# luoao-kddi/SCP

Hardware: AMD Instinct MI355X
Metric: KITTI frames/sec encode (SCP-EHEM, level 16) + bpp match vs ref (higher is better)
Workload: dtype f32 (dense layers and attention as bf16x3 split on bf16 MFMA, feature kNN as f16x3 split on f16 MFMA, fp32 accumulate; position kNN / CDF in fp32); 1 GPU; SCP-EHEM KITTI-like synthetic 120k-pt frames, --spher --mullevel lidar_level=16 (BASELINE.json configs[2]), seeded random weights; nodes_per_frame=577403, windows_per_frame=100, frames_per_gpu=46, frames_in_flight=4, frames_per_launch_sequence=1, transform=host-numpy on a prefetch thread (strict identity: the reference's integers), parallelism=frame-sharded x1, rank_cores=256, rank_cores_pinned=False

## Files before the change

include/scp.h:

```cpp
#ifndef SCP_H
#define SCP_H
#include <stddef.h>
#include <stdint.h>

#ifdef __cplusplus
extern "C" {
#endif

#define SCP_API __attribute__((visibility("default")))

#define SCP_OK 0
#define SCP_EINVAL (-1)
#define SCP_ENOMEM (-2)
#define SCP_ESMALL (-3)
#define SCP_EHIP (-4)
#define SCP_ESTATE (-5)

#define SCP_MAX_DEPTH 21
#define SCP_MAX_SEGMENTS 62

#define SCP_ABI_VERSION 220
SCP_API int scp_version(void);
SCP_API int scp_last_hip_error(void);
SCP_API int scp_device_count(void);
// ... 68 lines not shown
                                      uint8_t *sym_coded, int64_t *pos_mm, void *stream);

SCP_API int scp_geom_context_octattn(scp_geom *g, int32_t seg, uint8_t *ctx, float *pos, uint8_t *sym, void *stream);

SCP_API int scp_knn_topk(const float *x, int32_t B, int32_t n, int32_t C, int32_t k, int32_t *idx, void *stream);

SCP_API int scp_knn_topk_packed(const float *x, const int32_t *ctab, int32_t total_rows, int32_t C, int32_t *idx, void *stream);
SCP_API int scp_knn_topk_packed_bounded(const float *x, const int32_t *ctab, int32_t total_rows, int32_t C, const float *thr0,
                                int32_t *idx, void *stream);

SCP_API int scp_edge_gather_max(const float *u, const float *v, const int32_t *idx, const float *scale, const float *shift,
                        int32_t B, int32_t n, int32_t Cout, int32_t k, float *out, int32_t out_stride, void *stream);
SCP_API int scp_edge_gather_max_ld(const float *u, int64_t ldu, const float *v, int64_t ldv, const int32_t *idx, const float *scale,
                           const float *shift, int32_t B, int32_t n, int32_t Cout, int32_t k, float *out, int32_t out_stride,
                           void *stream);

SCP_API int scp_swin_attention(const float *q, const float *k, const float *v, const float *bias_table,
                       int32_t B, int32_t Lp, int32_t shift, int32_t ldq, int32_t ldkv, float *out, void *stream);

SCP_API int scp_split_weight_bf16(const float *W, int32_t N, int32_t K, int32_t Npad, int32_t Kpad, void *hi, void *lo, void *stream);
SCP_API int scp_linear_bf16x3(const float *A, int64_t lda, const void *Whi, const void *Wlo, int32_t Kpad, const float *bias,
                      const float *residual, int64_t ldr, float *C, int64_t ldc, int32_t M, int32_t N, int32_t K, int32_t act,
                      void *stream);

SCP_API int scp_split_weight_f16(const float *W, int32_t N, int32_t K, int32_t Npad, int32_t Kpad, void *hi, void *lo,
                                 float *inv_scale, void *stream);
SCP_API int scp_linear_f16x3(const float *A, int64_t lda, const void *Whi, const void *Wlo, const float *w_inv_scale, int32_t Kpad,
                             const float *bias, const float *residual, int64_t ldr, float *C, int64_t ldc, int32_t M, int32_t N,
                             int32_t K, int32_t act, float *row_scale_ws, void *stream);
SCP_API int scp_row_scale_f16(const float *A, int64_t lda, int32_t M, int32_t K, float *scale, float *inv_scale, void *stream);
SCP_API int scp_linear_f16x3_scaled(const float *A, int64_t lda, const void *Whi, const void *Wlo, const float *w_inv_scale, int32_t Kpad,
                                    const float *bias, const float *residual, int64_t ldr, float *C, int64_t ldc, int32_t M, int32_t N,
                                    int32_t K, int32_t act, const float *scale, const float *inv_scale, void *stream);

SCP_API int scp_tile_weight_bf16(const void *plane, int32_t Npad, int32_t Kpad, void *tiled, void *stream);
SCP_API int scp_split_rows_f16(const float *A, int64_t lda, int32_t M, int32_t K, void *hi, void *lo, int64_t ldp, float *scale, float *inv_scale,
                               void *stream);
SCP_API int scp_layernorm_add_split_f16(const float *a, const float *b, int64_t rows, int32_t C, const float *gamma, const float *beta, float eps,
                                        float *out, void *hi, void *lo, int64_t ldp, float *scale, float *inv_scale, void *stream);
SCP_API int scp_linear_split_f16(const void *Ahi, const void *Alo, int64_t lda, const float *a_inv_scale, const void *Whi, const void *Wlo,
                                 const float *w_inv_scale, int32_t Npad, int32_t Kpad, const float *bias, const float *residual, int64_t ldr,
                                 float *C, int64_t ldc, int32_t M, int32_t N, int32_t K, int32_t act, int32_t cfg, void *stream);
SCP_API int scp_linear_split_f16_max(const void *Ahi, const void *Alo, int64_t lda, const float *a_inv_scale, const void *Whi, const void *Wlo,
                                     const float *w_inv_scale, int32_t Npad, int32_t Kpad, const float *bias, const float *residual, int64_t ldr,
                                     float *C, int64_t ldc, int32_t M, int32_t N, int32_t K, int32_t act, int32_t cfg, uint32_t *row_max,
                                     uint32_t *col_max, int32_t col_lo, int32_t col_hi, int32_t col_rows, void *stream);
SCP_API int scp_row_scale_from_max(const uint32_t *row_max, int32_t M, float *scale, float *inv_scale, void *stream);
SCP_API int scp_linear_split(const void *Ahi, const void *Alo, int64_t lda, const void *Whi, const void *Wlo, int32_t Npad, int32_t Kpad,
                     const float *bias, const float *residual, int64_t ldr, float *C, int64_t ldc, void *Ohi, void *Olo, int64_t ldo,
                     int32_t M, int32_t N, int32_t K, int32_t act, int32_t cfg, void *stream);

SCP_API int scp_linear_split_gather(const void *Ahi, const void *Alo, int64_t lda, const void *Whi, const void *Wlo, int32_t Npad, int32_t Kpad,
                            const float *bias, const float *residual, int64_t ldr, const int64_t *res_map, float *C, int64_t ldc, void *Ohi,
                            void *Olo, int64_t ldo, int32_t M, int32_t N, int32_t K, int32_t act, int32_t cfg, void *stream);
SCP_API int scp_linear_split_hier2(const void *A0hi, const void *A0lo, int64_t lda0, int32_t K0pad, const void *A1hi, const void *A1lo, int64_t lda1,
                                   int64_t M1, const void *W0hi, const void *W0lo, const void *W1hi, const void *W1lo, int32_t Npad,
                                   const int64_t *parent, const float *bias, const float *res, int64_t ldr, const int64_t *res_map, void *Ohi,
                                   void *Olo, int64_t ldo, int32_t M, int32_t N, int32_t act, void *stream);
SCP_API int scp_linear_split_scatter(const void *Ahi, const void *Alo, int64_t lda, const void *Whi, const void *Wlo, int32_t Npad, int32_t Kpad,
                             const float *bias, const int64_t *out_map, float *C, int64_t ldc, int32_t M, int32_t N, int32_t K, int32_t act,
                             int32_t cfg, void *stream);
SCP_API int scp_split_rows(const float *src, int64_t ld_src, int64_t n_src, const int64_t *idx, int32_t C, void *hi, void *lo, int64_t ldo,
                   int64_t rows, void *stream);
SCP_API int scp_layernorm_rows_split(const float *x, int64_t ldx, int64_t n_src_rows, const int64_t *ia, const int64_t *ib, int32_t C,
                             const float *gamma, const float *beta, const float *valid, float eps, void *ohi, void *olo, int64_t ldo,
                             int64_t rows, void *stream);
SCP_API int scp_layernorm_add(const float *a, const float *b, int64_t rows, int32_t C, const float *gamma, const float *beta, float eps,
                              float *out, void *stream);
SCP_API int scp_swin_attention_packed_split(const float *q, const float *k, const float *v, const float *bias_table, const int32_t *wtab,
                                    int32_t total_windows, int32_t shift, int32_t ldq, int32_t ldkv, void *ohi, void *olo, int64_t ldo,
                                    void *stream);


SCP_API int scp_swin_attention_packed(const float *q, const float *k, const float *v, const float *bias_table, const int32_t *wtab,
                              int32_t total_windows, int32_t shift, int32_t ldq, int32_t ldkv, float *out, void *stream);

SCP_API int scp_layernorm_rows(const float *x, int64_t ldx, int64_t n_src_rows, const int64_t *ia, const int64_t *ib, int32_t C,
                       const float *gamma, const float *beta, const float *valid, float eps, float *out, int64_t ldo, int64_t rows,
                       void *stream);
SCP_API int scp_gather_rows(const float *src, int64_t lds, const int64_t *idx, int32_t C, float *out, int64_t ldo, int64_t rows, void *stream);

SCP_API int scp_linear_f32(const float *A, int64_t lda, const float *W, const float *bias, float *C, int64_t ldc, int32_t M, int32_t N, int32_t K,
                   int32_t act, void *stream);

SCP_API int scp_octattn_attention(const float *q_u, const float *k, const float *k_u, const float *v, const float *v_u,
                          int32_t B, int32_t c, int32_t H, int32_t hd, float *out, float *out_u, void *stream);

SCP_API int64_t scp_octattn_f16x3_ws_bytes(int32_t B, int32_t c, int32_t H);
SCP_API int scp_octattn_attention_f16x3(const float *q_u, const float *k, const float *k_u, const float *v, const float *v_u,
                                        int64_t ldkv, int32_t B, int32_t c, int32_t H, int32_t hd, float *out, float *out_u, void *workspace,
                                        int64_t ws_bytes, void *stream);
SCP_API int scp_octattn_attention_f16x3_vmax(const float *q_u, const float *k, const float *k_u, const float *v, const float *v_u,
                                             int64_t ldkv, int32_t B, int32_t c, int32_t H, int32_t hd, float *out, float *out_u, void *workspace,
                                             int64_t ws_bytes, const uint32_t *vmax_bits, void *stream);
SCP_API int scp_octattn_attention_rowinv(const float *q_u, int64_t qw, int64_t qr, const float *k, const float *v, int64_t kw, int64_t kr,
                                         const float *k_u, const float *v_u, int64_t uw, int64_t ur, float *out, float *out_u, int64_t ow,
                                         int64_t orr, int32_t B, int32_t q0, int32_t q1, int32_t qoff, int32_t H, int32_t hd, void *stream);
SCP_API int scp_octattn_attention_rowinv_step(const float *q_u, int64_t qr, const float *k, const float *v, int64_t kw, int64_t kr,
                                              int32_t slots, int32_t rows, const float *k_u, const float *v_u, int64_t ur, float *out,
                                              float *out_u, int64_t orr, const int32_t *t, const int32_t *slot, int32_t S, int32_t H,
                                              int32_t hd, void *stream);
SCP_API int scp_decode_expand_octattn(const int64_t *sym, const int64_t *cum, const uint8_t *ctx, const int32_t *apos, int64_t n, int32_t L,
                                      int32_t shift, int32_t depth, uint8_t *cctx, int32_t *capos, float *cpos, uint8_t *occ8, void *stream);
SCP_API int scp_octattn_embed(const uint8_t *ctx, const float *pos, int64_t n, int32_t c, const float *occ_enc, int32_t d_occ,
                              const float *level_enc, int32_t d_lvl, int32_t max_level, const float *octant_enc, int32_t d_oct,
                              const float *pos_w, const float *pos_b, int32_t d_pos, const float *pe, int32_t level_cap, float *E,
                              void *hi, void *lo, int64_t ldp, float *scale, float *inv_scale, void *stream);

SCP_API int scp_softmax_cdf(const float *logits, int64_t ld, int64_t n, int32_t nsym, const uint8_t *sym,
                    float *pmf, uint32_t *lohi, uint16_t *cdf_full, void *stream);
SCP_API int scp_pmf_cdf(const float *pmf, int64_t n, int32_t nsym, const uint8_t *sym, uint32_t *lohi,
                uint16_t *cdf_full, void *stream);

typedef struct scp_rate_seg {
    int64_t rows;
    double ideal_bits, table_bits;
    int64_t top1, bad_rows;
} scp_rate_seg;
SCP_API int64_t scp_rate_workspace_bytes(int64_t n, int32_t nseg);
SCP_API int scp_rate_segments(const float *logits, int64_t ld, int64_t n, int32_t nsym, const uint8_t *sym, const uint32_t *lohi,
                              const int64_t *seg_off, int32_t nseg, scp_rate_seg *out, double *row_ideal, double *row_table,
                              void *workspace, int64_t workspace_bytes, void *stream);

SCP_API int scp_ac_encode_cdf(const uint16_t *cdf, const int16_t *sym, int64_t n, int32_t Lp, uint8_t *out, size_t cap,
                      size_t *out_len);
SCP_API int scp_ac_encode_lohi(const uint32_t *lohi, int64_t n, uint8_t *out, size_t cap, size_t *out_len);
typedef struct scp_ac_dec scp_ac_dec;
SCP_API int scp_ac_dec_new(scp_ac_dec **d, const uint8_t *stream, size_t len, int32_t Lp);
SCP_API int scp_ac_dec_next(scp_ac_dec *d, const uint16_t *cdf_row);
SCP_API int scp_ac_dec_run(scp_ac_dec *d, const uint16_t *cdf, int64_t n, int16_t *out);
SCP_API int scp_ac_dec_free(scp_ac_dec *d);

typedef struct scp_legacy_node { uint32_t nodeid, octant, parent; uint8_t oct; uint32_t pos[3]; } scp_legacy_node;
SCP_API void *new_vector(void);
SCP_API void delete_vector(void *v);
SCP_API int vector_size(void *v);
SCP_API void *vector_get(void *v, int level);
SCP_API void vector_push_back(void *v, int i);
SCP_API void *genOctreeInterface(void *v, const double *xyz, int n);
SCP_API int Nodes_size(void *level);
SCP_API scp_legacy_node *Nodes_get(void *level, int i);
SCP_API int int_size(void *codes);
SCP_API int int_get(void *codes, int i);

SCP_API int scp_nn_sqdist_f64(const double *a, int64_t na, const double *b, int64_t nb, double *d2, void *stream);

enum { SCP_TIE_MEAN_NORMAL = 0, SCP_TIE_PLANE_ERROR = 1 };
SCP_API int scp_estimate_normals_f64(const double *xyz, int64_t n, double radius, int32_t max_nn, const double *view, double *normals,
                                     int32_t *count, int32_t *idx, void *stream);
SCP_API int scp_nn_tieset_f64(int32_t mode, const double *q, int64_t nq, const double *p, int64_t np, const double *dmin, const double *nrm,
                              double *out, void *stream);

#define SCP_DIST_MAX_RINGS 64
#define SCP_DIST_MAX_BINS 4096
#define SCP_DIST_MAX_POINTS (1ll << 30)
enum { SCP_DIST_FLAG_AXIS = 1, SCP_DIST_FLAG_GROUP_CLAMPED = 2, SCP_DIST_FLAG_NO_NEIGHBOUR = 4 };
typedef struct scp_dist_seg {
    int64_t rows, axis_rows;
    double sum_sq, sum_r2, sum_phi2, sum_theta2, sum_r, max_sq;
    int64_t hist[64];
} scp_dist_seg;
SCP_API int scp_nn_error_split_f64(const double *a, int64_t na, const double *b, int64_t nb, const double *view, const double *edges_sq,
                                   int32_t n_rings, const int32_t *group , int32_t n_groups, int32_t *idx_out, double *d2_out,
                                   double *comp_out , int32_t *bin_out, uint8_t *flag_out, void *stream);
SCP_API int scp_dist_segments_f64(const double *d2, const double *comp, const uint8_t *flag, const int64_t *order , int64_t n,
                                  const int64_t *seg_off, int32_t n_bins, scp_dist_seg *out, void *stream);

#define SCP_SHARE_MAX_NODES (1ll << 30)
typedef struct scp_share_seg {
    int64_t leaves;
    double ideal_bits, table_bits, max_ideal_bits;
} scp_share_seg;
SCP_API int64_t scp_rate_leaf_share_workspace_bytes(int64_t total_nodes, int32_t nseg);
SCP_API int scp_rate_leaf_share(const uint8_t *occ, const uint8_t *level, const int32_t *parent, int64_t total_nodes, const double *bits_ideal,
                                const double *bits_table, const int64_t *segs , int32_t nseg, int64_t total_leaves,
                                int64_t *leaves, double *cost_ideal, double *cost_table, void *workspace, int64_t workspace_bytes, void *stream);
SCP_API int scp_ring_bins_f64(const double *xyz, int64_t n, const double *view, const double *edges_sq, int32_t n_rings,
                              const int32_t *group , int32_t n_groups, int32_t *bin_out, uint8_t *flag_out , void *stream);
SCP_API int scp_share_segments_f64(const double *cost_ideal, const double *cost_table, const int64_t *order , int64_t n,
                                   const int64_t *seg_off, int32_t n_bins, scp_share_seg *out, void *stream);

SCP_API int scp_embed_gather(const uint8_t *ctx, const float *pos, const int64_t *inmap, int64_t n_tokens, const float *occ_enc,
                     const float *level_enc, const float *octant_enc, float *x, float *pos_out, int64_t *occ_self, int64_t rows,
                     void *stream);

SCP_API int scp_packed_plan_sizes(const int64_t *lengths, int32_t W, int64_t *rows_out);
SCP_API int scp_packed_plan(const int64_t *lengths, int32_t W, int64_t *tables_dev, void *const *outs, int32_t n_outs, void *stream);

SCP_API int scp_decode_expand(const int64_t *sym, const int64_t *cum, const int32_t *pos, const uint8_t *anc, const uint8_t *octant, int64_t n,
                              int32_t L, int32_t shift, int32_t lv_next, int32_t lv_clamp, int32_t polar, double mn, double den, int32_t *cpos,
                              uint8_t *canc, uint8_t *coct, uint8_t *cctx, float *cposn, uint8_t *occ8, void *stream);

typedef struct scp_expand_seg {
    int64_t first, count, cfirst, coded;
    int32_t L, shift, lv_next, lv_clamp, polar, reserved;
    double mn, den;
} scp_expand_seg;
SCP_API int scp_decode_expand_batch(const int64_t *sym, const int64_t *cum, const int32_t *pos, const uint8_t *anc, const uint8_t *octant,
                                    int64_t n, const scp_expand_seg *seg, int32_t S, int32_t cs, const int64_t *wbase, int32_t K, int64_t M,
                                    int64_t T, void *table_dev, int32_t *cpos, uint8_t *canc, uint8_t *coct, uint8_t *cctx, float *cposn,
                                    uint8_t *occ8, void *stream);

SCP_API int scp_swin_ln_linear(const float *x, int64_t ldx, const float *valid, const void *Whi, const void *Wlo, const float *bias,
                               const float *wbeta, float eps, float *out, int64_t ldo, int32_t M, int32_t N, void *stream);
SCP_API int scp_swin_post_attn(const void *Ohi, const void *Olo, int64_t ldo_in, const float *x, int64_t ldx, const void *W, const float *bp,
                               const float *b1, const float *b2, float eps, float *out, int64_t ldc, int32_t M, const int32_t *tile_list,
                               int32_t n_tiles, void *stream);
SCP_API int64_t scp_swin_post_attn_weight_bytes(void);
SCP_API double scp_gelu_prescale(void);

SCP_API int scp_swin_merge(const float *x, int64_t ldx, int64_t n_src, const int64_t *ia, const int64_t *ib, const void *W, const float *wbeta,
                           float eps, float *out, int64_t ldo, int32_t M, void *stream);

SCP_API int scp_geo_edge_mlps(const float *pos1, int64_t ld1, const float *pos2, int64_t ld2, const float *pos3, int64_t ld3, const void *W,
                              const float *bias, float *out, int64_t ldo, int32_t M, void *stream);
SCP_API int scp_mlp3_rows(const float *x, int64_t ldx, int64_t n_src, const int64_t *in_map, const void *W, const float *bias, float *out, int64_t ldo,
                          const int64_t *out_map, int32_t M, int32_t N, void *stream);

SCP_API int scp_swin_kv_planes(const float *k, const float *v, int64_t ldkv, int64_t rows, void *khi, void *klo, void *vthi, void *vtlo, void *stream);
SCP_API int scp_swin_ln_qkv(const float *x, int64_t ldx, const float *valid, const void *Whi, const void *Wlo, const float *bias, const float *wbeta,
                            float eps, float *q, int64_t ldq, void *planes, int64_t Tp, int32_t M, int32_t N, void *stream);
SCP_API int scp_swin_attention_packed_planes(const float *q, const void *khi, const void *klo, const void *vthi, const void *vtlo,
                                             const float *bias_table, const int32_t *wtab, int32_t total_windows, int32_t shift, int32_t ldq,
                                             float *out, void *ohi, void *olo, int64_t ldo, const float *valid, void *stream);

#ifdef __cplusplus
}
#endif
#endif
```

include/scp_debug.h:

```cpp
#ifndef SCP_DEBUG_H
#define SCP_DEBUG_H
#include "scp.h"

#ifdef __cplusplus
extern "C" {
#endif

SCP_API int scp_set_knn_mode(int32_t f16x3);
SCP_API int scp_set_attention_mode(int32_t bf16x3);

SCP_API int scp_set_knn_workgroup(int32_t shape);
SCP_API int scp_knn_debug_buffer(unsigned long long *dev_buf);
SCP_API int scp_rc_debug_buffer(unsigned long long *dev_buf);
SCP_API int scp_set_attention_variant(int32_t v);
SCP_API int scp_get_attention_variant(void);
SCP_API int scp_rc_set_grid(int32_t workgroups);
SCP_API int scp_rc_set_wide(int32_t mode);

enum {
    SCP_PROF_POST_ATTN = 1,
    SCP_PROF_LN_LINEAR = 2,
    SCP_PROF_ATTENTION = 3,
    SCP_PROF_KNN_FEAT = 4,
    SCP_PROF_KNN_POS = 5,
    SCP_PROF_GEMM_SPLIT = 6,
    SCP_PROF_EDGE_MLP = 7,
    SCP_PROF_MERGE = 8,
    SCP_PROF_EDGE_GATHER = 9,
    SCP_PROF_CDF = 10,
    SCP_PROF_GEMM_F32 = 11,
    SCP_PROF_GEMM_ROWS = 12,
    SCP_PROF_SPLIT_ROWS = 13,
    SCP_PROF_LAYERNORM = 14,
    SCP_PROF_OA_ATTENTION = 15,
    SCP_PROF_GEOM = 16,
    SCP_PROF_OTHER = 17,
    SCP_PROF_MLP3 = 18,
    SCP_PROF_RATE = 19,
    SCP_PROF_NTAGS = 20
};
SCP_API int scp_prof_enable(int32_t on);
SCP_API int scp_prof_count(void);
SCP_API int scp_prof_read(int32_t cap, int32_t *tags, float *ms, double *work);

#ifdef __cplusplus
}
#endif
#endif
```

scp_amd/csrc/fused.hip:

```cpp
#include "scp_internal.h"

typedef _Float16 sf16x4 __attribute__((ext_vector_type(4)));
typedef float f32x4 __attribute__((ext_vector_type(4)));
typedef __bf16 bf16x4 __attribute__((ext_vector_type(4)));

template <int NV>
__global__ __launch_bounds__(256) void layernorm_rows_kernel(const float *__restrict__ x, int64_t ldx, int64_t n_src_rows,
                                                            const int64_t *__restrict__ ia, const int64_t *__restrict__ ib,
                                                            const float *__restrict__ gamma, const float *__restrict__ beta,
                                                            const float *__restrict__ valid, float eps, float *__restrict__ out, int64_t ldo,
                                                            int64_t rows, __bf16 *__restrict__ ohi, __bf16 *__restrict__ olo) {
    constexpr int RPW = 4;
    constexpr int C = 256 * NV;
    const int lane = threadIdx.x & 63;
    const int64_t r0 = ((int64_t)blockIdx.x * 4 + (threadIdx.x >> 6)) * RPW;
    if (r0 >= rows) return;
    f32x4 v[RPW][NV];
#pragma unroll
    for (int i = 0; i < RPW; ++i) {
        const int64_t r = r0 + i < rows ? r0 + i : rows - 1;
#pragma unroll
        for (int p = 0; p < NV; ++p) {
            int64_t src = r;
            if (ia) src = (p == 0) ? ia[r] : ib[r];
// ... 124 lines not shown
            if (lane + 64 * p < nq) mx = fmaxf(fmaxf(mx, fmaxf(fabsf(v[p][0]), fabsf(v[p][1]))), fmaxf(fabsf(v[p][2]), fabsf(v[p][3])));
        for (int o = 32; o > 0; o >>= 1) mx = fmaxf(mx, __shfl_xor(mx, o));
        float sc, isc;
        scp_pow2_scale(mx, sc, isc);
        if (lane == 0) { psc[r] = sc; pisc[r] = isc; }
        const int nqp = ((C + 31) & ~31) >> 2;
#pragma unroll
        for (int p = 0; p < NP; ++p) {
            const int q = lane + 64 * p;
            if (q >= nqp) continue;
            sf16x4 h4, l4;
#pragma unroll
            for (int u = 0; u < 4; ++u) {
                const float x = (q < nq ? v[p][u] : 0.f) * sc;
                const _Float16 hh = (_Float16)x;
                h4[u] = hh;
                l4[u] = (_Float16)(x - (float)hh);
            }
            *(sf16x4 *)(phi + r * ldp + 4 * q) = h4;
            *(sf16x4 *)(plo + r * ldp + 4 * q) = l4;
        }
    }
}

extern "C" SCP_API int scp_layernorm_add(const float *a, const float *b, int64_t rows, int32_t C, const float *gamma, const float *beta, float eps,
                                         float *out, void *stream) {
    if (!a || !gamma || !beta || !out || rows < 0 || C <= 0 || (C & 3) || C > 1024 ||
        (((uintptr_t)a | (uintptr_t)b | (uintptr_t)out | (uintptr_t)gamma | (uintptr_t)beta) & 15))
        return SCP_EINVAL;
    if (rows == 0) return SCP_OK;
    const unsigned nb = (unsigned)cdiv64(rows, 4);
    hipStream_t st = (hipStream_t)stream;
    SCP_PROF(SCP_PROF_LAYERNORM, st, (b ? 12.0 : 8.0) * rows * C);
    if (C <= 256) hipLaunchKernelGGL(layernorm_add_kernel<1>, dim3(nb), dim3(256), 0, st, a, b, rows, C, gamma, beta, eps, out);
    else if (C <= 512) hipLaunchKernelGGL(layernorm_add_kernel<2>, dim3(nb), dim3(256), 0, st, a, b, rows, C, gamma, beta, eps, out);
    else if (C <= 768) hipLaunchKernelGGL(layernorm_add_kernel<3>, dim3(nb), dim3(256), 0, st, a, b, rows, C, gamma, beta, eps, out);
    else hipLaunchKernelGGL(layernorm_add_kernel<4>, dim3(nb), dim3(256), 0, st, a, b, rows, C, gamma, beta, eps, out);
    LAUNCH_CHECK();
    return SCP_OK;
}

extern "C" SCP_API int scp_layernorm_add_split_f16(const float *a, const float *b, int64_t rows, int32_t C, const float *gamma, const float *beta,
                                                   float eps, float *out, void *hi, void *lo, int64_t ldp, float *scale, float *inv_scale,
                                                   void *stream) {
    const int Cp = (C + 31) & ~31;
    if (!a || !gamma || !beta || !out || !hi || !lo || !scale || !inv_scale || rows < 0 || C <= 0 || (C & 3) || Cp > 1024 || ldp < Cp || (ldp & 7) ||
        (((uintptr_t)a | (uintptr_t)b | (uintptr_t)out | (uintptr_t)gamma | (uintptr_t)beta | (uintptr_t)hi | (uintptr_t)lo) & 15))
        return SCP_EINVAL;
    if (rows == 0) return SCP_OK;
    const unsigned nb = (unsigned)cdiv64(rows, 4);
    hipStream_t st = (hipStream_t)stream;
    SCP_PROF(SCP_PROF_LAYERNORM, st, (b ? 16.0 : 12.0) * rows * C);
#define GOP(NP_) hipLaunchKernelGGL((layernorm_add_kernel<NP_, true>), dim3(nb), dim3(256), 0, st, a, b, rows, C, gamma, beta, eps, out, (_Float16 *)hi, \
                                    (_Float16 *)lo, ldp, scale, inv_scale)
    if (Cp <= 256) GOP(1); else if (Cp <= 512) GOP(2); else if (Cp <= 768) GOP(3); else GOP(4);
#undef GOP
    LAUNCH_CHECK();
    return SCP_OK;
}

__global__ __launch_bounds__(256) void gather_rows_kernel(const float *__restrict__ src, int64_t lds, const int64_t *__restrict__ idx, int C4,
                                                         float *__restrict__ out, int64_t ldo, int64_t total ) {
    const int64_t g = (int64_t)blockIdx.x * 256 + threadIdx.x;
    if (g >= total) return;
    const int64_t r = g / C4;
    const int c = (int)(g - r * C4) * 4;
    *(f32x4 *)(out + r * ldo + c) = *(const f32x4 *)(src + idx[r] * lds + c);
}

extern "C" SCP_API int scp_gather_rows(const float *src, int64_t lds, const int64_t *idx, int32_t C, float *out, int64_t ldo, int64_t rows,
                                       void *stream) {
    if (!src || !idx || !out || rows < 0 || C <= 0 || (C & 3) || (lds & 3) || (ldo & 3) || (((uintptr_t)src | (uintptr_t)out) & 15)) return SCP_EINVAL;
    if (rows == 0) return SCP_OK;
    const int64_t total = rows * (C / 4);
    hipLaunchKernelGGL(gather_rows_kernel, dim3((unsigned)cdiv64(total, 256)), dim3(256), 0, (hipStream_t)stream, src, lds, idx, C / 4, out, ldo,
                       total);
    LAUNCH_CHECK();
    return SCP_OK;
}

__global__ __launch_bounds__(256) void embed_gather_kernel(const unsigned char *__restrict__ ctx, const float *__restrict__ pos,
                                                          const int64_t *__restrict__ inmap, int64_t n_tokens, const float *__restrict__ occ_enc,
                                                          const float *__restrict__ level_enc, const float *__restrict__ octant_enc,
                                                          float *__restrict__ x, float *__restrict__ pos_out, int64_t *__restrict__ occ_self,
                                                          int64_t rows) {
    const int64_t g = (int64_t)blockIdx.x * 256 + threadIdx.x;
    if (g >= rows * 20) return;
    const int64_t r = g / 20;
    const int p = (int)(g - r * 20);
    const int64_t t = inmap[r];
    const bool pad = t >= n_tokens;
    const unsigned char *c = ctx + (pad ? 0 : t) * 12;
    f32x4 v;
    if (p < 12) {
        const int a = p >> 2;
        const int occ = pad ? 255 : c[3 * a + 2];
        v = *(const f32x4 *)(occ_enc + occ * 16 + 4 * (p & 3));
    } else if (p < 16) {
        const int lv = pad ? 0 : c[3 * (p - 12)];
        v = *(const f32x4 *)(level_enc + lv * 4);
    } else {
        const int oc = pad ? 0 : c[3 * (p - 16) + 1];
        v = *(const f32x4 *)(octant_enc + oc * 4);
    }
    *(f32x4 *)(x + r * 80 + 4 * p) = v;
    if (p == 0) {
        occ_self[r] = pad ? 255 : c[11];
        pos_out[3 * r] = pad ? 0.f : pos[3 * t];
        pos_out[3 * r + 1] = pad ? 0.f : pos[3 * t + 1];
        pos_out[3 * r + 2] = pad ? 0.f : pos[3 * t + 2];
    }
}

extern "C" SCP_API int scp_embed_gather(const uint8_t *ctx, const float *pos, const int64_t *inmap, int64_t n_tokens, const float *occ_enc,
                                        const float *level_enc, const float *octant_enc, float *x, float *pos_out, int64_t *occ_self,
                                        int64_t rows, void *stream) {
    if (!ctx || !pos || !inmap || !occ_enc || !level_enc || !octant_enc || !x || !pos_out || !occ_self || rows < 0 || n_tokens <= 0 ||
        (((uintptr_t)occ_enc | (uintptr_t)level_enc | (uintptr_t)octant_enc | (uintptr_t)x) & 15))
        return SCP_EINVAL;
    if (rows == 0) return SCP_OK;
    hipLaunchKernelGGL(embed_gather_kernel, dim3((unsigned)cdiv64(rows * 20, 256)), dim3(256), 0, (hipStream_t)stream, ctx, pos, inmap, n_tokens,
                       occ_enc, level_enc, octant_enc, x, pos_out, occ_self, rows);
    LAUNCH_CHECK();
    return SCP_OK;
}
```

scp_amd/csrc/gemm.hip:

```cpp
#include "scp_internal.h"

typedef __bf16 bf16x8 __attribute__((ext_vector_type(8)));
typedef __bf16 bf16x4 __attribute__((ext_vector_type(4)));
typedef _Float16 f16x8 __attribute__((ext_vector_type(8)));
typedef _Float16 f16x4 __attribute__((ext_vector_type(4)));
typedef float f32x16 __attribute__((ext_vector_type(16)));
typedef float f32x4 __attribute__((ext_vector_type(4)));

#define BM 128
#define BN 128
#define BK 32
#define LDP 40

enum { ACT_NONE = 0, ACT_LEAKY = 1, ACT_GELU = 2, ACT_RELU = 3 };

template <int act>
__device__ __forceinline__ float apply_act(float y) {
    if (act == ACT_LEAKY) return y > 0.f ? y : 0.01f * y;
    if (act == ACT_GELU) return scp_gelu(y);
    if (act == ACT_RELU) return y > 0.f ? y : 0.f;
    return y;
}

template <int ACT, bool F16>
// ... 295 lines not shown
            }
            *(f16x4 *)(hi + (int64_t)(row0 + i) * ldp + k) = h4;
            *(f16x4 *)(lo + (int64_t)(row0 + i) * ldp + k) = l4;
        }
    }
}

extern "C" SCP_API int scp_split_rows_f16(const float *A, int64_t lda, int32_t M, int32_t K, void *hi, void *lo, int64_t ldp, float *scale,
                                          float *inv_scale, void *stream) {
    const int Kp = (K + 31) & ~31;
    if (!A || !hi || !lo || !scale || !inv_scale || M <= 0 || K <= 0 || (K & 3) || K > 1024 || (lda & 3) || lda < K || ldp < Kp || (ldp & 7) ||
        ((uintptr_t)A & 15) || (((uintptr_t)hi | (uintptr_t)lo) & 15))
        return SCP_EINVAL;
    const dim3 grid((unsigned)((M + 15) / 16));
    SCP_PROF(SCP_PROF_SPLIT_ROWS, stream, 8.0 * M * (double)K);
#define GOR(N_) hipLaunchKernelGGL((split_rows_f16_kernel<N_>), grid, dim3(256), 0, (hipStream_t)stream, A, lda, M, K, Kp, (_Float16 *)hi, (_Float16 *)lo, \
                                   ldp, scale, inv_scale)
    if (Kp <= 256) GOR(1); else if (Kp <= 512) GOR(2); else if (Kp <= 768) GOR(3); else GOR(4);
#undef GOR
    LAUNCH_CHECK();
    return SCP_OK;
}

__global__ __launch_bounds__(256) void row_scale_from_max_kernel(const unsigned *__restrict__ mxb, int M, float *__restrict__ sc, float *__restrict__ isc) {
    const int m = blockIdx.x * 256 + threadIdx.x;
    if (m >= M) return;
    float s, is;
    pow2_scale(__uint_as_float(mxb[m]), s, is);
    sc[m] = s; isc[m] = is;
}

extern "C" SCP_API int scp_row_scale_from_max(const uint32_t *row_max, int32_t M, float *scale, float *inv_scale, void *stream) {
    if (!row_max || !scale || !inv_scale || M <= 0) return SCP_EINVAL;
    hipLaunchKernelGGL(row_scale_from_max_kernel, dim3((unsigned)((M + 255) / 256)), dim3(256), 0, (hipStream_t)stream, (const unsigned *)row_max, M, scale, inv_scale);
    LAUNCH_CHECK();
    return SCP_OK;
}

extern "C" SCP_API int scp_row_scale_f16(const float *A, int64_t lda, int32_t M, int32_t K, float *scale, float *inv_scale, void *stream) {
    if (!A || !scale || !inv_scale || M <= 0 || K <= 0 || (K & 3) || (lda & 3) || lda < K || ((uintptr_t)A & 15)) return SCP_EINVAL;
    hipLaunchKernelGGL(row_scale_kernel, dim3((unsigned)((M + 15) / 16)), dim3(256), 0, (hipStream_t)stream, A, lda, M, K, scale, inv_scale);
    LAUNCH_CHECK();
    return SCP_OK;
}

static int linear_f16x3_launch(const float *A, int64_t lda, const void *Whi, const void *Wlo, const float *w_inv_scale, int32_t Kpad,
                               const float *bias, const float *residual, int64_t ldr, float *C, int64_t ldc, int32_t M, int32_t N, int32_t K,
                               int32_t act, float *sc, float *isc, bool compute_scales, void *stream) {
    if (!A || !Whi || !Wlo || !w_inv_scale || !C || !sc || !isc || M <= 0 || N <= 0 || K <= 0 || (K & 3) || (lda & 3) || Kpad < K ||
        (Kpad % BK) || act < 0 || act > 3 || ((uintptr_t)A & 15) || lda < K || ldc < N || (residual && ldr < N))
        return SCP_EINVAL;
    if (compute_scales) hipLaunchKernelGGL(row_scale_kernel, dim3((unsigned)((M + 15) / 16)), dim3(256), 0, (hipStream_t)stream, A, lda, M, K, sc, isc);
    const dim3 grid((unsigned)(((N + BN - 1) / BN) * ((M + BM - 1) / BM)));
    SCP_PROF(SCP_PROF_GEMM_ROWS, stream, 2.0 * M * (double)N * K);
#define GO(ACT) hipLaunchKernelGGL((gemm_bf16x3_kernel<ACT, true>), grid, dim3(512), 0, (hipStream_t)stream, A, lda, (const __bf16 *)Whi, \
                              (const __bf16 *)Wlo, Kpad, bias, residual, ldr, C, ldc, M, N, K, sc, isc, w_inv_scale, gemm_wtiled())
    switch (act) { case ACT_LEAKY: GO(ACT_LEAKY); break; case ACT_GELU: GO(ACT_GELU); break; case ACT_RELU: GO(ACT_RELU); break; default: GO(ACT_NONE); }
#undef GO
    LAUNCH_CHECK();
    return SCP_OK;
}

extern "C" SCP_API int scp_linear_f16x3(const float *A, int64_t lda, const void *Whi, const void *Wlo, const float *w_inv_scale,
                                        int32_t Kpad, const float *bias, const float *residual, int64_t ldr, float *C, int64_t ldc,
                                        int32_t M, int32_t N, int32_t K, int32_t act, float *row_scale_ws, void *stream) {
    if (!row_scale_ws) return SCP_EINVAL;
    return linear_f16x3_launch(A, lda, Whi, Wlo, w_inv_scale, Kpad, bias, residual, ldr, C, ldc, M, N, K, act, row_scale_ws, row_scale_ws + M, true,
                               stream);
}

extern "C" SCP_API int scp_linear_f16x3_scaled(const float *A, int64_t lda, const void *Whi, const void *Wlo, const float *w_inv_scale,
                                               int32_t Kpad, const float *bias, const float *residual, int64_t ldr, float *C, int64_t ldc,
                                               int32_t M, int32_t N, int32_t K, int32_t act, const float *scale, const float *inv_scale,
                                               void *stream) {
    return linear_f16x3_launch(A, lda, Whi, Wlo, w_inv_scale, Kpad, bias, residual, ldr, C, ldc, M, N, K, act, (float *)scale, (float *)inv_scale,
                               false, stream);
}

#define FBM 128
#define FBN 64
#define FBK 32
#define FLD 36

template <int ACT>
__global__ __launch_bounds__(256, 2) void gemm_f32_kernel(const float *__restrict__ A, int64_t lda, const float *__restrict__ W,
                                                         const float *__restrict__ bias, float *__restrict__ C, int64_t ldc, int M, int N, int K) {
    __shared__ __attribute__((aligned(16))) float sA[FBM * FLD];
    __shared__ __attribute__((aligned(16))) float sB[FBN * FLD];
    const int tid = threadIdx.x, w = tid >> 6, lane = tid & 63, col = lane & 31, h = lane >> 5;
    const int ntn = (N + FBN - 1) / FBN;
    const int m0 = (blockIdx.x / ntn) * FBM, n0 = (blockIdx.x % ntn) * FBN;
    f32x16 acc[2];
#pragma unroll
    for (int j = 0; j < 2; ++j)
#pragma unroll
        for (int r = 0; r < 16; ++r) acc[j][r] = 0.f;
    const int nk = (K + FBK - 1) / FBK;
    const bool vec = ((K & 3) == 0) && ((lda & 3) == 0) && ((((uintptr_t)A | (uintptr_t)W) & 15) == 0);
    const int pr = tid >> 3, pc = (tid & 7) * 4;
    f32x4 ra[4], rb[2];
    auto load_tile = [&](int kt) {
        const int kk = kt * FBK + pc;
        const bool kin = kk < K;
#pragma unroll
        for (int i = 0; i < 4; ++i) {
            const int m = m0 + pr + 32 * i;
            const int mc = m < M ? m : M - 1, kc = kin ? kk : 0;
            const f32x4 v = *(const f32x4 *)(A + (int64_t)mc * lda + kc);
            ra[i] = (kin && m < M) ? v : (f32x4){0.f, 0.f, 0.f, 0.f};
        }
#pragma unroll
        for (int i = 0; i < 2; ++i) {
            const int n = n0 + pr + 32 * i;
            const int nc = n < N ? n : N - 1, kc = kin ? kk : 0;
            const f32x4 v = *(const f32x4 *)(W + (int64_t)nc * K + kc);
            rb[i] = (kin && n < N) ? v : (f32x4){0.f, 0.f, 0.f, 0.f};
        }
    };
    auto store_tile = [&]() {
        const int o = pc >> 1;
#pragma unroll
        for (int i = 0; i < 4; ++i) {
            float *d = sA + (pr + 32 * i) * FLD;
            *(float2 *)(d + o) = make_float2(ra[i][0], ra[i][2]);
            *(float2 *)(d + 16 + o) = make_float2(ra[i][1], ra[i][3]);
        }
#pragma unroll
        for (int i = 0; i < 2; ++i) {
            float *d = sB + (pr + 32 * i) * FLD;
            *(float2 *)(d + o) = make_float2(rb[i][0], rb[i][2]);
            *(float2 *)(d + 16 + o) = make_float2(rb[i][1], rb[i][3]);
        }
    };
    if (vec) load_tile(0);
    for (int kt = 0; kt < nk; ++kt) {
        const int k0 = kt * FBK;
        __syncthreads();
        if (vec) {
            store_tile();
        } else {
        for (int e = tid; e < FBM * FBK; e += 256) {
            const int r = e >> 5, k = e & 31;
            const int m = m0 + r, kk = k0 + k;
            sA[r * FLD + (k & 1) * 16 + (k >> 1)] = (m < M && kk < K) ? A[(int64_t)m * lda + kk] : 0.f;
        }
        for (int e = tid; e < FBN * FBK; e += 256) {
            const int r = e >> 5, k = e & 31;
            const int n = n0 + r, kk = k0 + k;
            sB[r * FLD + (k & 1) * 16 + (k >> 1)] = (n < N && kk < K) ? W[(int64_t)n * K + kk] : 0.f;
        }
        }
        __syncthreads();
        if (vec && kt + 1 < nk) load_tile(kt + 1);
        const float *ar = sA + (w * 32 + col) * FLD + h * 16;
#pragma unroll
        for (int g = 0; g < 4; ++g) {
            const f32x4 a = *(const f32x4 *)(ar + 4 * g);
#pragma unroll
            for (int j = 0; j < 2; ++j) {
                const f32x4 b = *(const f32x4 *)(sB + (j * 32 + col) * FLD + h * 16 + 4 * g);
                acc[j] = __builtin_amdgcn_mfma_f32_32x32x2f32(a[0], b[0], acc[j], 0, 0, 0);
                acc[j] = __builtin_amdgcn_mfma_f32_32x32x2f32(a[1], b[1], acc[j], 0, 0, 0);
                acc[j] = __builtin_amdgcn_mfma_f32_32x32x2f32(a[2], b[2], acc[j], 0, 0, 0);
                acc[j] = __builtin_amdgcn_mfma_f32_32x32x2f32(a[3], b[3], acc[j], 0, 0, 0);
            }
        }
    }
#pragma unroll
    for (int j = 0; j < 2; ++j) {
        const int n = n0 + j * 32 + col;
        if (n >= N) continue;
        const float bv = bias ? bias[n] : 0.f;
#pragma unroll
        for (int r = 0; r < 16; ++r) {
            const int m = m0 + w * 32 + (r & 3) + 8 * (r >> 2) + 4 * h;
            if (m < M) C[(int64_t)m * ldc + n] = apply_act<ACT>(acc[j][r] + bv);
        }
    }
}

extern "C" SCP_API int scp_linear_f32(const float *A, int64_t lda, const float *W, const float *bias, float *C, int64_t ldc, int32_t M, int32_t N,
                                      int32_t K, int32_t act, void *stream) {
    if (!A || !W || !C || M <= 0 || N <= 0 || K <= 0 || lda < K || ldc < N || act < 0 || act > 3) return SCP_EINVAL;
    const dim3 grid((unsigned)(((N + FBN - 1) / FBN) * ((M + FBM - 1) / FBM)));
    SCP_PROF(SCP_PROF_GEMM_F32, stream, 2.0 * M * (double)N * K);
#define GOF(ACT) hipLaunchKernelGGL(gemm_f32_kernel<ACT>, grid, dim3(256), 0, (hipStream_t)stream, A, lda, W, bias, C, ldc, M, N, K)
    switch (act) { case ACT_LEAKY: GOF(ACT_LEAKY); break; case ACT_GELU: GOF(ACT_GELU); break; case ACT_RELU: GOF(ACT_RELU); break; default: GOF(ACT_NONE); }
#undef GOF
    LAUNCH_CHECK();
    return SCP_OK;
}
```

scp_amd/csrc/lnlin2.hip:

```cpp
#include <stdlib.h>
#include <type_traits>
#include "rc_common.h"

#define L2_Q 16384
#define L2_OFF_BOUNCE (3 * L2_Q)
#define L2_OFF_BIAS (L2_OFF_BOUNCE + 4 * RC_BOUNCE)
#define L2_LDS (L2_OFF_BIAS + 8192)
static_assert(L2_LDS <= 80 * 1024, "two workgroups per CU: at most half of the 160 KiB");
#define L2_LDS_ONE (160 * 1024)

__device__ __forceinline__ void l2_issue(const RcLane &L, __amdgpu_buffer_rsrc_t wr_hi, __amdgpu_buffer_rsrc_t wr_lo, int j, int qt, char *dst) {
#pragma unroll
    for (int i = 0; i < 4; ++i) {
        const int b = i >> 1, plane = i & 1;
        const int soff = ((2 * j + b) * 16 + (L.w >> 1) * 8 + qt * 2 + (L.w & 1)) * 1024;
        __builtin_amdgcn_raw_ptr_buffer_load_lds(plane ? wr_lo : wr_hi, (rc_lds_ptr_t)(dst + (L.w + 4 * i) * 1024), 16, L.lane * 16, soff, 0, 0);
    }
}

#define L2_READ4(d0, d1, d2, d3, addr, o0, o1, o2, o3)                                                                                  \
    asm volatile("ds_read_b128 %0, %4 offset:%5\n\tds_read_b128 %1, %4 offset:%6\n\tds_read_b128 %2, %4 offset:%7\n\t"                      \
                 "ds_read_b128 %3, %4 offset:%8\n\ts_waitcnt lgkmcnt(0)"                                                                  \
                 : "=&v"(d0), "=&v"(d1), "=&v"(d2), "=&v"(d3) : "v"(addr), "n"(o0), "n"(o1), "n"(o2), "n"(o3) : "memory")
#define L2_READ4_AHEAD(d0, d1, d2, d3, addr, o0, o1, o2, o3)                                                                            \
// ... 7 lines not shown
__device__ __forceinline__ void l2_quarter(unsigned ad0, unsigned ad1, rf32x16 &c0, rf32x16 &c1, const rbf16x8 (&Xh)[16], const rbf16x8 (&Xl)[16]) {
#define L2_MFMA(c, wf, xf) c = SWAP ? __builtin_amdgcn_mfma_f32_32x32x16_bf16(xf, wf, c, 0, 0, 0) : __builtin_amdgcn_mfma_f32_32x32x16_bf16(wf, xf, c, 0, 0, 0)
#define L2_FRAGS(M, A, ad, s) M(A[1], A[3], A[0], A[2], ad, 4096 + ((s) >> 1) * 1024, 12288 + ((s) >> 1) * 1024, ((s) >> 1) * 1024, 8192 + ((s) >> 1) * 1024)
    rbf16x8 A[2][4];
    L2_FRAGS(L2_READ4, A[0], ad0, 0);
#pragma unroll
    for (int s = 0; s < 4; ++s) {
        const int k = 4 * Q + s, n = (s + 1) & 1;
        if (s < 3) {
            if (n) L2_FRAGS(L2_READ4_AHEAD, A[1], ad1, s + 1);
            else L2_FRAGS(L2_READ4_AHEAD, A[0], ad0, s + 1);
        }
        __builtin_amdgcn_sched_barrier(0);
        L2_MFMA(c0, A[s & 1][1], Xh[k]);
        L2_MFMA(c1, A[s & 1][3], Xh[k]);
        L2_MFMA(c0, A[s & 1][0], Xl[k]);
        L2_MFMA(c1, A[s & 1][2], Xl[k]);
        L2_MFMA(c0, A[s & 1][0], Xh[k]);
        L2_MFMA(c1, A[s & 1][2], Xh[k]);
        __builtin_amdgcn_sched_barrier(0);
        if (s < 3) L2_WAIT4(A[n][0], A[n][1], A[n][2], A[n][3]);
    }
#undef L2_FRAGS
#undef L2_MFMA
}

__device__ __forceinline__ unsigned l2_split_pair(float x0, float x1, int plane) {
    const unsigned hh = rc_pack2(x0, x1);
    return plane ? rc_pack2(x0 - __builtin_bit_cast(float, hh << 16), x1 - __builtin_bit_cast(float, hh & 0xffff0000u)) : hh;
}

__device__ __forceinline__ void l2_store_k(const RcLane &L, char *bounce, const rf32x16 &c0, const rf32x16 &c1, __amdgpu_buffer_rsrc_t prs, int kvoff,
                                           int pbytes, int head) {
    ri32x4 y[2][4];
    int col = L.col;
    asm volatile("" : "+v"(col));
#pragma unroll
    for (int plane = 0; plane < 2; ++plane) {
#pragma unroll
        for (int b = 0; b < 2; ++b)
#pragma unroll
            for (int q = 0; q < 4; ++q) {
                const rf32x16 &c = b ? c1 : c0;
                *(ru32x2 *)(bounce + col * 128 + (((4 * b + q) ^ (col & 7)) << 4) + 8 * L.h) =
                    (ru32x2){l2_split_pair(c[4 * q], c[4 * q + 1], plane), l2_split_pair(c[4 * q + 2], c[4 * q + 3], plane)};
            }
#pragma unroll
        for (int it = 0; it < 4; ++it) y[plane][it] = *(const ri32x4 *)(bounce + it * 1024 + L.lane * 16);
    }
#pragma unroll
    for (int plane = 0; plane < 2; ++plane)
#pragma unroll
        for (int it = 0; it < 4; ++it)
            __builtin_amdgcn_raw_buffer_store_b128(y[plane][it], prs, kvoff, it * 8 * 512 + head * 128 + plane * pbytes, 0);
    asm volatile("s_waitcnt lgkmcnt(0)" ::: "memory");
}

__device__ __forceinline__ void l2_store_v(const RcLane &L, char *bounce, const rf32x16 &c0, const rf32x16 &c1, __amdgpu_buffer_rsrc_t prs, int vblk,
                                           int pbytes, int head) {
    ri32x4 y[2][4];
    int col = L.col;
    asm volatile("" : "+v"(col));
#pragma unroll
    for (int plane = 0; plane < 2; ++plane) {
#pragma unroll
        for (int b = 0; b < 2; ++b)
#pragma unroll
            for (int cc = 0; cc < 2; ++cc) {
                const rf32x16 &c = b ? c1 : c0;
                const int d = col + 32 * b, R = d >> 1, sl = (d & 1) * 4 + 2 * cc + L.h;
                *(ru32x4 *)(bounce + R * 128 + ((sl ^ (R & 7)) << 4)) =
                    (ru32x4){l2_split_pair(c[8 * cc], c[8 * cc + 1], plane), l2_split_pair(c[8 * cc + 2], c[8 * cc + 3], plane),
                             l2_split_pair(c[8 * cc + 4], c[8 * cc + 5], plane), l2_split_pair(c[8 * cc + 6], c[8 * cc + 7], plane)};
            }
#pragma unroll
        for (int it = 0; it < 4; ++it) y[plane][it] = *(const ri32x4 *)(bounce + it * 1024 + L.lane * 16);
    }
#pragma unroll
    for (int plane = 0; plane < 2; ++plane)
#pragma unroll
        for (int it = 0; it < 4; ++it)
            __builtin_amdgcn_raw_buffer_store_b128(y[plane][it], prs, L.lane * 16, it * 1024 + (vblk + head) * 4096 + (2 + plane) * pbytes, 0);
    asm volatile("s_waitcnt lgkmcnt(0)" ::: "memory");
}

template <bool KV>
__global__ __launch_bounds__(256, 2) void ln2_proj_kernel(const RcLnLinArgs a) {
    extern __shared__ __attribute__((aligned(1024))) char smem[];
    const RcLane L = rc_lane();
    const int ntiles = (a.M + RC_ROWS - 1) / RC_ROWS;
    const int nsteps = a.N >> 6;
    const int nq = KV ? a.nq : nsteps;
    char *bounce = smem + L2_OFF_BOUNCE + L.w * RC_BOUNCE;
    const unsigned ab = (unsigned)(uintptr_t)(rc_lds_ptr_t)smem + L.rg * 2048;
    const unsigned af0 = ab + L.frag, af1 = ab + (L.frag ^ 32);
    const unsigned asb = (unsigned)(uintptr_t)(rc_lds_ptr_t)(smem + L2_OFF_BIAS);
    const int ldo_bytes = (int)(a.ldo * 4);
    const int voff = (32 * L.w + (L.lane >> 3)) * ldo_bytes + (L.lane & 7) * 16;
    const int pbytes = (int)a.plane_bytes;
    const __amdgpu_buffer_rsrc_t prs = __builtin_amdgcn_make_buffer_rsrc((void *)a.planes, 0, (KV && !(a.probe & 1)) ? (int)(4 * a.plane_bytes) : 0, 0x00020000);
    const bool dma = !(a.probe & 2);

    const int wbytes = ((a.N + 255) & ~255) * 512;
    const __amdgpu_buffer_rsrc_t wr_hi = __builtin_amdgcn_make_buffer_rsrc((void *)a.Whi, 0, wbytes, 0x00020000);
    const __amdgpu_buffer_rsrc_t wr_lo = __builtin_amdgcn_make_buffer_rsrc((void *)a.Wlo, 0, wbytes, 0x00020000);

    float *sb = (float *)(smem + L2_OFF_BIAS), *sbw = sb + 1024;
    for (int i = threadIdx.x; i < a.N; i += 256) {
        const float b = a.bias ? a.bias[i] : 0.f;
        sb[i] = b; sbw[i] = b + (a.wbeta ? a.wbeta[i] : 0.f);
    }
    __syncthreads();
    int slot = 0;
    if (dma) { l2_issue(L, wr_hi, wr_lo, 0, 0, smem); l2_issue(L, wr_hi, wr_lo, 0, 1, smem + L2_Q); }
    for (int tile = blockIdx.x; tile < ntiles; tile += (int)gridDim.x) {
        const int m0 = tile * RC_ROWS;
        const int row = m0 + 32 * L.w + L.col;
        const int rowc = row < a.M ? row : a.M - 1;
        float keep = (row < a.M) ? 1.0f : 0.0f;
        if (a.valid) keep *= a.valid[rowc];
        rbf16x8 Xh[16], Xl[16];
        {
            float v[128];
            const float *src = a.x + (int64_t)((a.probe & 4) ? (rowc & 127) % a.M : rowc) * a.ldx + 8 * L.h;
#pragma unroll
            for (int s = 0; s < 16; ++s) {
                const rf32x4 q0 = *(const rf32x4 *)(src + 16 * s), q1 = *(const rf32x4 *)(src + 16 * s + 4);
#pragma unroll
                for (int u = 0; u < 4; ++u) { v[8 * s + u] = q0[u]; v[8 * s + 4 + u] = q1[u]; }
            }
            float mean, rstd;
            rc_ln_stats(v, a.eps, mean, rstd);
            const float sc = rstd * keep;
#pragma unroll
            for (int s = 0; s < 16; ++s) {
                float f[8];
#pragma unroll
                for (int i = 0; i < 8; ++i) f[i] = (v[8 * s + i] - mean) * sc;
                rc_split8(f, Xh[s], Xl[s]);
            }
        }
        const bool kept = keep != 0.f;
        const int64_t rows_left = (int64_t)a.M - m0;
        const int64_t span = (rows_left < RC_ROWS ? rows_left : RC_ROWS) * a.ldo * 4;
        const __amdgpu_buffer_rsrc_t rs = __builtin_amdgcn_make_buffer_rsrc(a.out + (int64_t)m0 * a.ldo, 0, (a.probe & 1) ? 0 : (int)span, 0x00020000);
        const unsigned kmask = (unsigned)__builtin_amdgcn_ballot_w64(kept);
        const unsigned maskh = kmask >> (4 * L.h);
        const int kvoff = (m0 + 32 * L.w + (L.lane >> 3)) * 512 + (L.lane & 7) * 16;
        const int vblk = ((m0 >> 5) + L.w) * 4;

        const unsigned atb = asb + (kept ? 4096 : 0) + 16 * L.h, atv = asb + 4 * L.col;
        rf32x16 c0, c1;
        auto bias_start = [&](int j) {
            if (KV && j >= nq + 4) {
                float bb[2], bwv[2];
                const unsigned ad = atv + 256 * j;
                asm volatile("ds_read_b32 %0, %4\n\tds_read_b32 %1, %4 offset:128\n\tds_read_b32 %2, %4 offset:4096\n\tds_read_b32 %3, %4 offset:4224\n\t"
                             "s_waitcnt lgkmcnt(0)" : "=&v"(bb[0]), "=&v"(bb[1]), "=&v"(bwv[0]), "=&v"(bwv[1]) : "v"(ad) : "memory");
#pragma unroll
                for (int blk = 0; blk < 2; ++blk) {
                    rf32x16 &c = blk ? c1 : c0;
#pragma unroll
                    for (int r = 0; r < 16; ++r) c[r] = ((maskh >> (8 * (r >> 2) + (r & 3))) & 1u) ? bwv[blk] : bb[blk];
                }
            } else {
                const unsigned ad = atb + 256 * j;
                rf32x4 t[2][4];
                L2_READ4(t[0][0], t[0][1], t[0][2], t[0][3], ad, 0, 32, 64, 96);
                L2_READ4(t[1][0], t[1][1], t[1][2], t[1][3], ad, 128, 160, 192, 224);
#pragma unroll
                for (int q = 0; q < 4; ++q)
#pragma unroll
                    for (int u = 0; u < 4; ++u) { c0[4 * q + u] = t[0][q][u]; c1[4 * q + u] = t[1][q][u]; }
            }
        };
        bias_start(0);
        SCP_WAIT_DMA(0);
        auto steps = [&](auto sw, int ja, int jb) {
        constexpr bool SW = decltype(sw)::value;
        for (int j = ja; j < jb; ++j) {
            const int jn = j + 1 < nsteps ? j + 1 : 0;
#define L2_QUARTER(Q, N)                                                                                                                \
            {                                                                                                                           \
                L2_TOP(N);                                                                                                              \
                const int sl2 = slot == 0 ? 2 : slot - 1;                    \
                if (dma) l2_issue(L, wr_hi, wr_lo, Q < 2 ? j : jn, (Q + 2) & 3, smem + sl2 * L2_Q);                                       \
                __builtin_amdgcn_sched_barrier(0);                                                                                      \
                const unsigned a0 = af0 + slot * L2_Q, a1 = af1 + slot * L2_Q;                                                          \
                l2_quarter<SW, Q>(a0, a1, c0, c1, Xh, Xl);                                                                              \
                slot = slot == 2 ? 0 : slot + 1;                                                                                        \
            }
            L2_QUARTER(0, 12)
            L2_QUARTER(1, 12)
            L2_QUARTER(2, 4)
            L2_QUARTER(3, 4)
#undef L2_QUARTER
            __builtin_amdgcn_sched_barrier(0);
            if (!SW && j < nq) {
#pragma unroll
                for (int blk = 0; blk < 2; ++blk) {
                    rf32x4 o[4];
#pragma unroll
                    for (int q = 0; q < 4; ++q)
#pragma unroll
                        for (int u = 0; u < 4; ++u) o[q][u] = (blk ? c1 : c0)[4 * q + u];
                    rc_store_block(L, bounce, o, rs, ldo_bytes, voff, 64 * j + 32 * blk);
                }
            } else if (!SW) {
                l2_store_k(L, bounce, c0, c1, prs, kvoff, pbytes, j - nq);
            } else {
                l2_store_v(L, bounce, c0, c1, prs, vblk, pbytes, j - nq - 4);
            }
            if (j + 1 < nsteps) bias_start(jn);
        }
        };
        if (KV) { steps(std::false_type(), 0, nq + 4); steps(std::true_type(), nq + 4, nsteps); }
        else steps(std::false_type(), 0, nsteps);
    }
    SCP_WAIT_DMA(0);
}

int scp_lnlin2_mode() {
    static int mode = -1;
    if (mode < 0) { const char *e = getenv("SCP_LNLIN"); mode = e ? atoi(e) : 0; if (mode < 0 || mode > 2) mode = 0; }
    return mode;
}

int scp_lnlin2_launch(RcLnLinArgs a, bool kv, int ncu, hipStream_t stream) {
    static int one = -1, probe = -1;
    if (one < 0) { const char *e = getenv("SCP_LNLIN_ONE"); one = (e && e[0] == '1') ? 1 : 0; }
    if (probe < 0) { const char *e = getenv("SCP_RC_PROBE"); probe = e ? atoi(e) : 0; }
    static bool configured = false;
    if (!configured) {
        HIP_TRY(hipFuncSetAttribute((const void *)ln2_proj_kernel<false>, hipFuncAttributeMaxDynamicSharedMemorySize, one ? L2_LDS_ONE : L2_LDS));
        HIP_TRY(hipFuncSetAttribute((const void *)ln2_proj_kernel<true>, hipFuncAttributeMaxDynamicSharedMemorySize, one ? L2_LDS_ONE : L2_LDS));
        configured = true;
    }
    a.ngroups = 1; a.probe = probe; a.dbg = nullptr;
    const int ntiles = (a.M + RC_ROWS - 1) / RC_ROWS;
    const int wgs = (one ? 1 : 2) * ncu;
    const dim3 grid((unsigned)(ntiles < wgs ? ntiles : wgs));
    if (kv) hipLaunchKernelGGL(ln2_proj_kernel<true>, grid, dim3(256), one ? L2_LDS_ONE : L2_LDS, stream, a);
    else hipLaunchKernelGGL(ln2_proj_kernel<false>, grid, dim3(256), one ? L2_LDS_ONE : L2_LDS, stream, a);
    LAUNCH_CHECK();
    return SCP_OK;
}
```

scp_amd/csrc/rc_common.h:

```cpp
#pragma once
#include "scp_internal.h"

typedef __bf16 rbf16x8 __attribute__((ext_vector_type(8)));
typedef float rf32x16 __attribute__((ext_vector_type(16)));
typedef float rf32x4 __attribute__((ext_vector_type(4)));
typedef int ri32x4 __attribute__((ext_vector_type(4)));
typedef __attribute__((address_space(3))) void *rc_lds_ptr_t;
typedef const __attribute__((address_space(1))) void *rc_glb_ptr_t;

#define RC_ROWS 128
#define RC_BOUNCE 4096

__device__ __forceinline__ void rc_dma16(const void *g, char *l) {
    __builtin_amdgcn_global_load_lds((rc_glb_ptr_t)g, (rc_lds_ptr_t)l, 16, 0, 0);
}

typedef float rf32x2 __attribute__((ext_vector_type(2)));
typedef __bf16 rbf16x2 __attribute__((ext_vector_type(2)));
typedef unsigned ru32x4 __attribute__((ext_vector_type(4)));
typedef unsigned ru32x2 __attribute__((ext_vector_type(2)));
__device__ __forceinline__ unsigned rc_pack2(float a, float b) {
    const rf32x2 v = {a, b};
    return __builtin_bit_cast(unsigned, __builtin_convertvector(v, rbf16x2));
}
__device__ __forceinline__ void rc_split2(float a, float b, unsigned &hi, unsigned &lo) {
    asm volatile("" : "+v"(a), "+v"(b));
    hi = rc_pack2(a, b);
    lo = rc_pack2(a - __builtin_bit_cast(float, hi << 16), b - __builtin_bit_cast(float, hi & 0xffff0000u));
}
__device__ __forceinline__ void rc_split8(const float *f, rbf16x8 &hi, rbf16x8 &lo) {
    ru32x4 h, l;
#pragma unroll
    for (int i = 0; i < 4; ++i) { unsigned a, b; rc_split2(f[2 * i], f[2 * i + 1], a, b); h[i] = a; l[i] = b; }
    hi = __builtin_bit_cast(rbf16x8, h);
    lo = __builtin_bit_cast(rbf16x8, l);
}

struct RcLane {
    int lane, col, h, w;
    int frag;
    int rg;
};

__device__ __forceinline__ RcLane rc_lane() {
    RcLane L;
    const int tid = threadIdx.x;
    L.lane = tid & 63; L.col = L.lane & 31; L.h = L.lane >> 5;
    L.w = __builtin_amdgcn_readfirstlane(tid >> 6);
    L.frag = (L.col & 15) * 64 + ((L.h ^ ((L.col >> 2) & 3)) << 4);
    L.rg = L.col >> 4;
    return L;
}

__device__ __forceinline__ void rc_store_block(const RcLane &L, char *bounce, const rf32x4 v[4], __amdgpu_buffer_rsrc_t rs, int ldo_bytes, int voff,
                                               int ch0) {
#pragma unroll
    for (int q = 0; q < 4; ++q)
        *(rf32x4 *)(bounce + L.col * 128 + (((2 * q + L.h) ^ (L.col & 7)) << 4)) = v[q];
    asm volatile("s_waitcnt lgkmcnt(0)" ::: "memory");
    rf32x4 y[4];
#pragma unroll
    for (int it = 0; it < 4; ++it) {
        const int rho = 8 * it + (L.lane >> 3), kap = L.lane & 7;
        y[it] = *(const rf32x4 *)(bounce + rho * 128 + ((kap ^ (rho & 7)) << 4));
    }
#pragma unroll
    for (int it = 0; it < 4; ++it) __builtin_amdgcn_raw_buffer_store_b128(__builtin_bit_cast(ri32x4, y[it]), rs, voff, it * 8 * ldo_bytes + ch0 * 4, 0);
    asm volatile("s_waitcnt lgkmcnt(0)" ::: "memory");
}

__device__ __forceinline__ void rc_ln_stats(const float *v , float eps, float &mean, float &rstd) {
    float s = 0.f;
#pragma unroll
    for (int i = 0; i < 128; i += 4) s += (v[i] + v[i + 1]) + (v[i + 2] + v[i + 3]);
    s += __shfl_xor(s, 32);
    mean = s * (1.0f / 256.0f);
    float q = 0.f;
#pragma unroll
    for (int i = 0; i < 128; ++i) { const float d = v[i] - mean; q += d * d; }
    q += __shfl_xor(q, 32);
    rstd = rsqrtf(q * (1.0f / 256.0f) + eps);
}

struct RcLnLinArgs {
    const float *x; int64_t ldx;
    const float *valid;
    const __bf16 *Whi, *Wlo;
    const float *bias, *wbeta;
    float *out; int64_t ldo;
    int M, N;
    float eps;
    int probe;
    unsigned long long *dbg;
    __bf16 *planes; int64_t plane_bytes; int nq;
    int ngroups;
};

int scp_lnlin2_mode();
int scp_lnlin2_launch(RcLnLinArgs a, bool kv, int ncu, hipStream_t stream);
```

scp_amd/csrc/rowchain.hip:

```cpp
#include <stdlib.h>
#include "scp_internal.h"
#include "rc_common.h"

#define RC_SLOT 32768
#define RC_RING (4 * RC_SLOT)
#define RC_OFF_BOUNCE RC_RING
#define RC_OFF_BIAS (RC_RING + 4 * RC_BOUNCE)
#define RC_LDS (RC_OFF_BIAS + 16384)

__device__ __forceinline__ void rc_issue_rowchunk(const RcLane &L, const __bf16 *Whi, const __bf16 *Wlo, int g, char *slot) {
#pragma unroll
    for (int j = 0; j < 4; ++j) {
        const int p = L.w + 4 * j;
        const int64_t off = ((int64_t)g * 16 + p) * 512 + L.lane * 8;
        rc_dma16(Whi + off, slot + p * 1024);
        rc_dma16(Wlo + off, slot + 16384 + p * 1024);
    }
}

__device__ __forceinline__ void rc_issue_kchunk(const RcLane &L, const __bf16 *Whi, const __bf16 *Wlo, int c, int nks, char *slot) {
#pragma unroll
    for (int j = 0; j < 4; ++j) {
        const int p = L.w + 4 * j;
        const int64_t off = ((int64_t)p * nks + c) * 512 + L.lane * 8;
// ... 1393 lines not shown
            for (int q = 0; q < 4; ++q) {
                rf32x4 v;
#pragma unroll
                for (int u = 0; u < 4; ++u) v[u] = c[4 * q + u];
                *(rf32x4 *)(bounce + L.col * 128 + (((2 * q + L.h) ^ (L.col & 7)) << 4)) = v;
            }
            asm volatile("s_waitcnt lgkmcnt(0)" ::: "memory");
            rf32x4 y[4];
#pragma unroll
            for (int it = 0; it < 4; ++it) {
                const int rho = 8 * it + (L.lane >> 3);
                y[it] = *(const rf32x4 *)(bounce + rho * 128 + ((kap ^ (rho & 7)) << 4));
            }
            asm volatile("s_waitcnt lgkmcnt(0)" ::: "memory");
#pragma unroll
            for (int it = 0; it < 4; ++it)
                if (orow[it] && ch0 + 4 * kap < a.N) *(rf32x4 *)(orow[it] + ch0) = y[it];
        };
        for (int g = 0; g < 4; ++g) {
            RC_BIAS3(2)
            RC_STEP3()
            store_block(c0, 64 * g);
            store_block(c1, 64 * g + 32);
        }
#undef RC_LAYER3
#undef RC_BIAS3
#undef RC_STEP3
    }
    SCP_WAIT_DMA(0);
}

extern "C" SCP_API double scp_gelu_prescale(void) { return (double)SCP_GELU_S; }

static int rc_ll_groups(int ntiles, int nsteps, int ncu) {
    static int on = -1;
    if (on < 0) { const char *e = getenv("SCP_RC_GROUPS"); on = (e && e[0] == '0') ? 0 : 1; }
    int best = 1;
    if (on)
        for (int g = 2; g <= nsteps / 2; ++g)
            if ((nsteps / 2) % g == 0 && (int64_t)ntiles * g <= ncu) best = g;
    return best;
}

static unsigned long long *g_rc_dbg = nullptr;
extern "C" SCP_API int scp_rc_debug_buffer(unsigned long long *dev_buf) { g_rc_dbg = dev_buf; return SCP_OK; }

static int g_rc_num_cu = 0, g_rc_grid = 0;
static int g_rc_wide = -2;
static int rc_wide_mode() {
    if (g_rc_wide == -2) { const char *e = getenv("SCP_RC_WIDE"); g_rc_wide = e ? atoi(e) : -1; if (g_rc_wide < -1 || g_rc_wide > 1) g_rc_wide = -1; }
    return g_rc_wide;
}
extern "C" SCP_API int scp_rc_set_wide(int32_t mode) { g_rc_wide = (mode < -1 || mode > 1) ? -1 : mode; return SCP_OK; }
extern "C" SCP_API int scp_rc_set_grid(int32_t workgroups) { g_rc_grid = workgroups > 0 ? workgroups : 0; return SCP_OK; }
static int rc_num_cu() {
    if (g_rc_grid) return g_rc_grid;
    if (!g_rc_num_cu) {
        int dev = 0;
        hipDeviceProp_t p;
        if (hipGetDevice(&dev) != hipSuccess || hipGetDeviceProperties(&p, dev) != hipSuccess) return 256;
        g_rc_num_cu = p.multiProcessorCount > 0 ? p.multiProcessorCount : 256;
    }
    return g_rc_num_cu;
}

static bool rc_lnlin2_here(int ntiles, int ncu) {
    const int mode = scp_lnlin2_mode();
    return mode == 2 || (mode == 0 && 4 * (int64_t)ntiles >= 3 * (int64_t)ncu);
}

extern "C" SCP_API int scp_swin_ln_linear(const float *x, int64_t ldx, const float *valid, const void *Whi, const void *Wlo, const float *bias,
                                          const float *wbeta, float eps, float *out, int64_t ldo, int32_t M, int32_t N, void *stream) {
    if (!x || !Whi || !Wlo || !out || M <= 0 || N <= 0 || (N & 127) || N > 1024 || ldx < 256 || (ldx & 3) || ldo < N || (ldo & 3) ||
        (((uintptr_t)x | (uintptr_t)out | (uintptr_t)Whi | (uintptr_t)Wlo) & 15) || (int64_t)RC_ROWS * ldo * 4 > 0x7fffffffLL)
        return SCP_EINVAL;
    static bool configured = false;
    if (!configured) {
        HIP_TRY(hipFuncSetAttribute((const void *)rc_ln_linear_kernel<0>, hipFuncAttributeMaxDynamicSharedMemorySize, RC_LDS));
        configured = true;
    }
    RcLnLinArgs a;
    a.x = x; a.ldx = ldx; a.valid = valid; a.Whi = (const __bf16 *)Whi; a.Wlo = (const __bf16 *)Wlo; a.bias = bias; a.wbeta = wbeta;
    a.out = out; a.ldo = ldo; a.M = M; a.N = N; a.eps = eps;
    a.planes = nullptr; a.plane_bytes = 0; a.nq = 0;
    { static int pr = -1; if (pr < 0) { const char *e = getenv("SCP_RC_PROBE"); pr = e ? atoi(e) : 0; } a.probe = pr; }
    if (a.probe) { const char *e = getenv("SCP_RC_PROBE"); a.probe = e ? atoi(e) : 0; }
    a.dbg = g_rc_dbg;
    const int ntiles = (M + RC_ROWS - 1) / RC_ROWS;
    const int ncu = rc_num_cu();
    SCP_PROF(SCP_PROF_LN_LINEAR, stream, 2.0 * M * 256.0 * N);
    if (rc_lnlin2_here(ntiles, ncu)) return scp_lnlin2_launch(a, false, ncu, (hipStream_t)stream);
    a.ngroups = rc_ll_groups(ntiles, N / 64, ncu);
    hipLaunchKernelGGL(rc_ln_linear_kernel<0>, dim3((unsigned)(a.ngroups > 1 ? ntiles * a.ngroups : (ntiles < ncu ? ntiles : ncu))), dim3(256), RC_LDS, (hipStream_t)stream, a);
    LAUNCH_CHECK();
    return SCP_OK;
}

extern "C" SCP_API int scp_swin_ln_qkv(const float *x, int64_t ldx, const float *valid, const void *Whi, const void *Wlo, const float *bias,
                                       const float *wbeta, float eps, float *q, int64_t ldq, void *planes, int64_t Tp, int32_t M, int32_t N, void *stream) {
    if (!x || !Whi || !Wlo || !planes || M <= 0 || (M & 127) || (N != 768 && N != 512) || (N == 768 && (!q || ldq < 256 || (ldq & 3))) || ldx < 256 ||
        (ldx & 3) || Tp < M || (Tp & 31) || (((uintptr_t)x | (uintptr_t)q | (uintptr_t)Whi | (uintptr_t)Wlo | (uintptr_t)planes) & 15) ||
        (q && (int64_t)RC_ROWS * ldq * 4 > 0x7fffffffLL) || 4 * Tp * 512 > 0x7fffffffLL)
        return SCP_EINVAL;
    static bool configured = false;
    if (!configured) {
        HIP_TRY(hipFuncSetAttribute((const void *)rc_ln_linear_kernel<0, true>, hipFuncAttributeMaxDynamicSharedMemorySize, RC_LDS));
        configured = true;
    }
    RcLnLinArgs a;
    a.x = x; a.ldx = ldx; a.valid = valid; a.Whi = (const __bf16 *)Whi; a.Wlo = (const __bf16 *)Wlo; a.bias = bias; a.wbeta = wbeta;
    a.out = q; a.ldo = q ? ldq : 256; a.M = M; a.N = N; a.eps = eps; a.probe = 0; a.dbg = nullptr;
    a.planes = (__bf16 *)planes; a.plane_bytes = Tp * 512; a.nq = N / 64 - 8;
    const int ntiles = M / RC_ROWS, ncu = rc_num_cu();
    SCP_PROF(SCP_PROF_LN_LINEAR, stream, 2.0 * M * 256.0 * N);
    if (rc_lnlin2_here(ntiles, ncu)) return scp_lnlin2_launch(a, true, ncu, (hipStream_t)stream);
    a.ngroups = rc_ll_groups(ntiles, N / 64, ncu);
    hipLaunchKernelGGL((rc_ln_linear_kernel<0, true>), dim3((unsigned)(a.ngroups > 1 ? ntiles * a.ngroups : (ntiles < ncu ? ntiles : ncu))), dim3(256), RC_LDS, (hipStream_t)stream, a);
    LAUNCH_CHECK();
    return SCP_OK;
}

extern "C" SCP_API int scp_swin_post_attn(const void *Ohi, const void *Olo, int64_t ldo_in, const float *x, int64_t ldx, const void *W, const float *bp,
                                          const float *b1, const float *b2, float eps, float *out, int64_t ldc, int32_t M, const int32_t *tile_list,
                                          int32_t n_tiles, void *stream) {
    if (!Ohi || !Olo || !x || !W || !bp || !b1 || !b2 || !out || M <= 0 || (tile_list && (n_tiles <= 0 || n_tiles > (M + RC_ROWS - 1) / RC_ROWS)) || ldo_in < 256 || (ldo_in & 7) || ldx < 256 || (ldx & 3) || ldc < 256 ||
        (ldc & 3) || (((uintptr_t)Ohi | (uintptr_t)Olo | (uintptr_t)x | (uintptr_t)out | (uintptr_t)W) & 15) ||
        (int64_t)RC_ROWS * ldc * 4 > 0x7fffffffLL)
        return SCP_EINVAL;
    static bool configured = false;
    if (!configured) {
        HIP_TRY(hipFuncSetAttribute((const void *)rc_post_attn_kernel, hipFuncAttributeMaxDynamicSharedMemorySize, RC_LDS));
        HIP_TRY(hipFuncSetAttribute((const void *)rc_post_attn_wide_kernel, hipFuncAttributeMaxDynamicSharedMemorySize, RC_LDS));
        configured = true;
    }
    RcPostArgs a;
    a.Ohi = (const __bf16 *)Ohi; a.Olo = (const __bf16 *)Olo; a.ldo_in = ldo_in; a.x = x; a.ldx = ldx; a.W = W;
    a.bp = bp; a.b1 = b1; a.b2 = b2; a.out = out; a.ldc = ldc; a.M = M; a.eps = eps;
    a.dbg = g_rc_dbg;
    { const char *e = getenv("SCP_RC_DUMP"); a.dbg_mode = e ? atoi(e) : 0; }
    a.tile_list = tile_list; a.n_list = tile_list ? n_tiles : 0;
    const int ntiles = tile_list ? n_tiles : (M + RC_ROWS - 1) / RC_ROWS;
    const int ncu = rc_num_cu();
    SCP_PROF(SCP_PROF_POST_ATTN, stream, 2.0 * (tile_list ? (double)n_tiles * RC_ROWS : (double)M) * (256.0 * 256.0 + 2.0 * 256.0 * 1024.0));
    if (rc_wide_mode() == 1 || (rc_wide_mode() < 0 && !g_rc_dbg && !a.dbg_mode && 4 * (int64_t)ntiles <= (int64_t)ncu)) {
        const int items = 4 * ntiles;
        hipLaunchKernelGGL(rc_post_attn_wide_kernel, dim3((unsigned)(items < 2 * ncu ? items : 2 * ncu)), dim3(256), RC_LDS, (hipStream_t)stream, a);
        LAUNCH_CHECK();
        return SCP_OK;
    }
    hipLaunchKernelGGL(rc_post_attn_kernel, dim3((unsigned)(ntiles < ncu ? ntiles : ncu)), dim3(256), RC_LDS, (hipStream_t)stream, a);
    LAUNCH_CHECK();
    return SCP_OK;
}

extern "C" SCP_API int64_t scp_swin_post_attn_weight_bytes(void) { return 2 * (int64_t)RC_W_PLANE; }

extern "C" SCP_API int scp_geo_edge_mlps(const float *pos1, int64_t ld1, const float *pos2, int64_t ld2, const float *pos3, int64_t ld3, const void *W,
                                         const float *bias, float *out, int64_t ldo, int32_t M, void *stream) {
    if (!pos1 || !pos2 || !pos3 || !W || !bias || !out || M <= 0 || ld1 < 64 || ld2 < 128 || ld3 < 256 || ((ld1 | ld2 | ld3) & 3) || ldo < 128 || (ldo & 3) ||
        (((uintptr_t)pos1 | (uintptr_t)pos2 | (uintptr_t)pos3 | (uintptr_t)out | (uintptr_t)W) & 15) || (int64_t)RC_ROWS * ldo * 4 > 0x7fffffffLL)
        return SCP_EINVAL;
    static bool configured = false;
    if (!configured) {
        HIP_TRY(hipFuncSetAttribute((const void *)rc_edge_mlp_kernel, hipFuncAttributeMaxDynamicSharedMemorySize, RC_LDS));
        configured = true;
    }
    RcEdgeArgs a;
    a.p1 = pos1; a.p2 = pos2; a.p3 = pos3; a.ld1 = ld1; a.ld2 = ld2; a.ld3 = ld3; a.W = W; a.bias = bias; a.out = out; a.ldo = ldo; a.M = M;
    const int ntiles = (M + RC_ROWS - 1) / RC_ROWS, ncu = rc_num_cu();
    SCP_PROF(SCP_PROF_EDGE_MLP, stream, 2.0 * M * (448.0 * 256 + 2.0 * 256 * 256 + 512.0 * 256 + 256.0 * 256 + 256.0 * 128));
    hipLaunchKernelGGL(rc_edge_mlp_kernel, dim3((unsigned)(ntiles < ncu ? ntiles : ncu)), dim3(256), RC_LDS, (hipStream_t)stream, a);
    LAUNCH_CHECK();
    return SCP_OK;
}

extern "C" SCP_API int scp_mlp3_rows(const float *x, int64_t ldx, int64_t n_src, const int64_t *in_map, const void *W, const float *bias, float *out, int64_t ldo,
                                     const int64_t *out_map, int32_t M, int32_t N, void *stream) {
    if (!x || !W || !bias || !out || M <= 0 || n_src <= 0 || N <= 0 || N > 256 || (N & 3) || ldx < 256 || (ldx & 3) || ldo < N || (ldo & 3) ||
        (((uintptr_t)x | (uintptr_t)out | (uintptr_t)W) & 15))
        return SCP_EINVAL;
    static bool configured = false;
    if (!configured) {
        HIP_TRY(hipFuncSetAttribute((const void *)rc_mlp3_kernel, hipFuncAttributeMaxDynamicSharedMemorySize, RC_LDS));
        configured = true;
    }
    RcMlp3Args a;
    a.x = x; a.ldx = ldx; a.in_map = in_map; a.n_src = n_src; a.W = W; a.bias = bias; a.out = out; a.ldo = ldo; a.out_map = out_map; a.M = M; a.N = N;
    const int ntiles = (M + RC_ROWS - 1) / RC_ROWS, ncu = rc_num_cu();
    SCP_PROF(SCP_PROF_MLP3, stream, 2.0 * M * 3.0 * 256.0 * 256.0);
    hipLaunchKernelGGL(rc_mlp3_kernel, dim3((unsigned)(ntiles < ncu ? ntiles : ncu)), dim3(256), RC_LDS, (hipStream_t)stream, a);
    LAUNCH_CHECK();
    return SCP_OK;
}

extern "C" SCP_API int scp_swin_merge(const float *x, int64_t ldx, int64_t n_src, const int64_t *ia, const int64_t *ib, const void *W, const float *wbeta,
// ... 18 lines not shown
```

scp_amd/models/packed.py:

```python
import numpy as np
import torch
import torch.nn.functional as F

from .. import native
from ..ops import linear_s, leaky_mlp3_s, split_cat, linear, layer_norm, leaky_mlp3, _split, derived, frozen_epoch
from .ehem import SHIFT, WINDOW, _edge_conv_packed, qkv_fused


def _ceil512(a):
    return (a + WINDOW - 1) // WINDOW * WINDOW


def _tokens(L):
    wid = torch.repeat_interleave(torch.arange(L.numel(), device=L.device), L)
    first = torch.cumsum(L, 0) - L
    return wid, torch.arange(int(L.sum()), device=L.device) - first[wid]


class StageLayout:

    def __init__(self, L):
        self.L = L
        self.Lp = _ceil512(L)
        self.base = torch.cumsum(self.Lp, 0) - self.Lp
# ... 171 lines not shown
                query = _merge(stage.downsample, query, merges[s])
    return hs


def _concat(hs, cmaps, extra=None):
    n = len(hs) - 1 + (1 if extra is not None else 0)
    out = native.SplitAct.empty(hs[1].shape[0], 256 * n, hs[1].device)
    native.split_rows(hs[1], out=out.cols(0, 256))
    for s in range(1, len(hs) - 1):
        native.split_rows(hs[s + 1], idx=cmaps[s - 1], out=out.cols(256 * s, 256 * (s + 1)))
    if extra is not None:
        k = len(hs) - 1
        native.split_rows(extra[0], idx=extra[1], out=out.cols(256 * k, 256 * (k + 1)))
    return out


HIER = True


FUSE2 = __import__("os").environ.get("SCP_CONCAT_FUSE2", "1")[:1] != "0"


def _concat_layer(lin, hs, parents, extra=None, grand=None, a0_pre=None):
    n = len(hs) - 1
    def build():
        W = lin.weight.detach()
        slabs = [W[:, 256 * s:256 * (s + 1)].contiguous() for s in range(n)]
        if extra is not None:
            slabs[0] = torch.cat((slabs[0], W[:, 256 * n:256 * (n + 1)]), 1).contiguous()
        return slabs
    cache = derived(lin, "slabs+" if extra is not None else "slabs", (lin.weight,), build)
    fused = FUSE2 and n >= 3 and grand is not None and native.WTILE and hs[1].shape[0] % 256 == 0
    z = None
    for s in range(n - 1, 1 if fused else 0, -1):
        z = linear_s(native.split_rows(hs[s + 1]), cache[s], None, residual=z, res_map=None if z is None else parents[s], res_first=z is not None)
    if a0_pre is not None:
        native.split_rows(hs[1], out=a0_pre.cols(0, 256))
        a0 = a0_pre
    else:
        a0 = native.split_rows(hs[1]) if extra is None else split_cat((hs[1], extra))
    if fused:
        return native.linear_split_hier2(a0, _split(cache[0]), native.split_rows(hs[2]), _split(cache[1]), parents[0], lin.bias, native.ACT_LEAKY,
                                         residual=z, res_map=grand)
    return linear_s(a0, cache[0], lin.bias, act="leaky", residual=z, res_map=None if z is None else parents[0], res_first=z is not None,
                    want="split")


def _mlp_over_concat(seq, hs, parents, extra=None, grand=None, a0_pre=None):
    a = _concat_layer(seq[0], hs, parents, extra, grand, a0_pre)
    a = linear_s(a, seq[2].weight, seq[2].bias, act="leaky", want="split")
    return linear_s(a, seq[4].weight, seq[4].bias)


CHAIN_HEADS = __import__("os").environ.get("SCP_HEADS", "chain") != "split"


def _mlp3_weights(owner, name, seq):
    return derived(owner, "mlp3_" + name, [seq[i].weight for i in (0, 2, 4)] + [seq[i].bias for i in (0, 2, 4)], lambda: native.Mlp3Weights(seq))


def _head3(model, name, a, out=None, out_map=None, ncols=None):
    seq = getattr(model, name)
    N = seq[4].weight.shape[0]
    if CHAIN_HEADS:
        if out is None:
            out = torch.empty((a.shape[0], -(-N // 4) * 4), dtype=torch.float32, device=a.device)
        native.mlp3_rows(a, _mlp3_weights(model, name, seq), out, out_map=out_map, ncols=ncols)
        return out[:, :N] if out_map is None else None
    sa = native.split_rows(a)
    if out_map is not None:
        sa = linear_s(sa, seq[0].weight, seq[0].bias, act="leaky", want="split")
        sa = linear_s(sa, seq[2].weight, seq[2].bias, act="leaky", want="split")
        native.linear_split_scatter(sa, _split(seq[4].weight), seq[4].bias, out_map, out)
        return None
    return leaky_mlp3_s(seq, sa, out=out)


def _head_to_table(model, a, out_map, table):
    if CHAIN_HEADS and table.stride(0) < 256:
        raise native.ScpError("the coding-order table must have rows of at least 256 floats")
    _head3(model, "prob_pred_mlp1", a, out=table, out_map=out_map)


@torch.no_grad()
def ehem_phase1_packed(model, ctx, pos, plan, table=None):
    d = plan.d
    g = model.geo_feat_generator
    dev = ctx.device
    fused_in = (ctx.dtype == torch.uint8 and g.occ_enc.weight.shape[1] == 16 and g.level_enc.weight.shape[1] == 4
                and g.octant_enc.weight.shape[1] == 4)
    if fused_in:
        x, pos0, occ_self = native.embed_gather(ctx, pos, d["inmap"], g.occ_enc.weight, g.level_enc.weight, g.octant_enc.weight)
        P0 = x.shape[0]
    else:
        pad_ctx = torch.tensor([[0, 0, 255] * 4], dtype=ctx.dtype, device=dev)
        ctx0 = torch.cat((ctx, pad_ctx))[d["inmap"]].long()
        pos0 = torch.cat((pos, torch.zeros((1, 3), dtype=pos.dtype, device=dev)))[d["inmap"]].contiguous()
        P0 = ctx0.shape[0]
        x = torch.cat((F.embedding(ctx0[:, 2:11:3], g.occ_enc.weight).reshape(P0, -1),
                       F.embedding(ctx0[:, 0::3], g.level_enc.weight).reshape(P0, -1),
                       F.embedding(ctx0[:, 1::3], g.octant_enc.weight).reshape(P0, -1)), 1)
        occ_self = ctx0[:, 11]
    ktab = d["knn_tab"]
    c1, c2 = g.conv1[0].weight.shape[0], g.conv2[0].weight.shape[0]
    f2 = torch.empty((P0, c1 + x.shape[1]), dtype=torch.float32, device=dev)
    f2[:, c1:] = x
    pos1 = _edge_conv_packed(g.conv1, pos0, ktab, out=f2[:, :c1])
    x = leaky_mlp3(g.mlp2, x, exact=True)
    f3 = torch.empty((P0, c2 + x.shape[1]), dtype=torch.float32, device=dev)
    f3[:, c2:] = x
    pos2 = _edge_conv_packed(g.conv2, f2, ktab, out=f3[:, :c2])
    pos3 = _edge_conv_packed(g.conv3, f3, ktab, feeds_knn=False)
    nx = g.mlp3[4].weight.shape[0]
    feat = torch.empty((P0, nx + g.edge_mlp2[4].weight.shape[0]), dtype=torch.float32, device=dev)
    leaky_mlp3_s(g.mlp3, native.split_rows(x), out=feat[:, :nx])
    if (pos1.shape[1], pos2.shape[1], pos3.shape[1]) != (64, 128, 256) or feat.shape[1] - nx != 128:
        raise native.ScpError("GeoFeatGenerator: edge features of 64 / 128 / 256 channels expected (models/dgcnn.py:74-119)")
    ew = derived(g, "rowchain_edge", [l.weight for l in (g.edge_mlp1[0], g.edge_mlp1[2], g.edge_mlp1[4], g.edge_mlp2[0], g.edge_mlp2[2], g.edge_mlp2[4])] +
                 [l.bias for l in (g.edge_mlp1[0], g.edge_mlp1[2], g.edge_mlp1[4], g.edge_mlp2[0], g.edge_mlp2[2], g.edge_mlp2[4])],
                 lambda: native.EdgeMlpWeights(g.edge_mlp1, g.edge_mlp2))
    native.geo_edge_mlps(pos1, pos2, pos3, ew, feat[:, nx:])
    hs = _encoder(model.swin_self_transformer, feat, d["self_valid"], d["self_tab"], d["self_merge"], tiles=d.get("self_tiles"))
    feat_a = _mlp_over_concat(model.ancient_mlp, hs, d["self_parent"], grand=d["self_concat"][1]) if HIER else leaky_mlp3_s(model.ancient_mlp, _concat(hs, d["self_concat"]))
    Q0 = d["a1map"].shape[0]
    a1 = native.gather_rows(feat_a, d["a1map"], torch.empty((Q0, 256), dtype=torch.float32, device=dev))
    a2 = native.gather_rows(feat_a, d["a2map"], torch.empty((Q0, 256), dtype=torch.float32, device=dev))
    st = dict(a1=a1, a2=a2, pre_occ=occ_self[d["a1map"]])
    if table is not None:
        _head_to_table(model, a1, d["even_out"], table)
        return None, st
    prob1 = _head3(model, "prob_pred_mlp1", a1)
    return prob1[d["even_rows"]], st


@torch.no_grad()
def ehem_phase2_prepare(model, st, plan):
    d = plan.d
    a1, a2 = st["a1"], st["a2"]
    no = model.pre_occ_mlp[4].weight.shape[0]
    pre = torch.empty((a2.shape[0], no + model.pre_attn_mlp[4].weight.shape[0]), dtype=torch.float32, device=a2.device)
    _head3(model, "pre_attn_mlp", a1, out=pre[:, no:])
    enc = model.swin_cross_transformer
    qs, query = [], a2
    for s, stage in enumerate(enc.layers):
        v1 = d["cross_valid"][s].reshape(-1)
        row = []
        for blk in stage.blocks:
            w, _, qbias, eps_b, _ = _block_consts(blk, True)
            row.append(native.swin_ln_linear(query, w["q"], qbias, eps_b, v1))
        qs.append(row)
        if s < len(enc.layers) - 1:
            query = _merge(stage.downsample, query, d["cross_merge"][s])
    a0 = native.SplitAct.empty(a2.shape[0], 512, a2.device)
    native.split_rows(a2, out=a0.cols(256, 512))
    return dict(pre=pre, q=qs, a0=a0)


def phase2_prep_window(prep, bases, rows):
    return dict(pre=prep["pre"][bases[0]:bases[0] + rows[0]], q=[[q[bases[s]:bases[s] + rows[s]] for q in qs] for s, qs in enumerate(prep["q"])],
                a0=native.SplitAct(prep["a0"].t[:, bases[0]:bases[0] + rows[0]], prep["a0"].K))


@torch.no_grad()
def ehem_phase2_packed(model, st, plan, pre_occ=None, table=None, prep=None):
    d = plan.d
    g = model.geo_feat_generator
    a1, a2 = st["a1"], st["a2"]
    po = st["pre_occ"] if pre_occ is None else pre_occ
    lut = derived(model, "pre_occ_lut", [g.occ_enc.weight] + [model.pre_occ_mlp[i].weight for i in (0, 2, 4)] + [model.pre_occ_mlp[i].bias for i in (0, 2, 4)],
                  lambda: leaky_mlp3(model.pre_occ_mlp, g.occ_enc.weight.detach()).contiguous())
    no = lut.shape[1]
    if prep is not None:
        pre = prep["pre"]
    else:
        pre = torch.empty((a2.shape[0], no + model.pre_attn_mlp[4].weight.shape[0]), dtype=torch.float32, device=a2.device)
        _head3(model, "pre_attn_mlp", a1, out=pre[:, no:])
    native.gather_rows(lut, po, pre[:, :no])
    hc = _encoder(model.swin_cross_transformer, pre, d["cross_valid"], d["cross_tab"], d["cross_merge"], query=a2, tiles=d.get("cross_tiles"),
                  q_pre=None if prep is None else prep["q"])
    if table is not None:
        a = _concat_layer(model.prob_pred_mlp2[0], hc, d["cross_parent"], a2, d["cross_concat"][1], None if prep is None else prep.get("a0")) if HIER else linear_s(_concat(hc, d["cross_concat"], extra=(a2, None)), model.prob_pred_mlp2[0].weight, model.prob_pred_mlp2[0].bias, act="leaky", want="split")
        from ..ops import _split
        a = linear_s(a, model.prob_pred_mlp2[2].weight, model.prob_pred_mlp2[2].bias, act="leaky", want="split")
        native.linear_split_scatter(a, _split(model.prob_pred_mlp2[4].weight), model.prob_pred_mlp2[4].bias, d["odd_out"], table)
        return None
    prob2 = (_mlp_over_concat(model.prob_pred_mlp2, hc, d["cross_parent"], extra=a2, grand=d["cross_concat"][1], a0_pre=None if prep is None else prep.get("a0")) if HIER
             else leaky_mlp3_s(model.prob_pred_mlp2, _concat(hc, d["cross_concat"], extra=(a2, None))))
    return prob2[d["odd_rows"]]


@torch.no_grad()
def ehem_forward_packed(model, ctx, pos, plan, table=None):
    ev, st = ehem_phase1_packed(model, ctx, pos, plan, table=table)
# ... 2 lines not shown
```

scp_amd/native.py:

```python
import ctypes as C
import os

import numpy as np
import torch

HERE = os.path.dirname(os.path.abspath(__file__))
LIB_PATH = os.path.join(HERE, "libscp_hip.so")
MAX_DEPTH = 21

CART, SPHER, CYLIN = 0, 1, 2
POS_MINMAX, POS_MINMAX_MUL, POS_POW2 = 0, 1, 2
_ERR = {-1: "SCP_EINVAL", -2: "SCP_ENOMEM", -3: "SCP_ESMALL", -4: "SCP_EHIP", -5: "SCP_ESTATE"}


class ScpError(RuntimeError):
    pass


class QuantInfo(C.Structure):
    _fields_ = [("bin_num", C.c_double), ("qs", C.c_double * 3), ("offset", C.c_double * 3),
                ("max_coord", C.c_int32), ("min_coord", C.c_int32)]


class Segment(C.Structure):
    _fields_ = [("point_begin", C.c_int64), ("point_count", C.c_int64), ("path_len", C.c_int32),
                ("path_bits", C.c_int32), ("drop_last", C.c_int32), ("reserved", C.c_int32)]


class SegmentInfo(C.Structure):
    _fields_ = [("depth", C.c_int32), ("max_coord", C.c_int32), ("n_leaves", C.c_int64), ("n_nodes", C.c_int64),
                ("node_base", C.c_int64), ("level_count", C.c_int64 * (MAX_DEPTH + 1))]


_lib = None
_vp = C.c_void_p


ABI_VERSION = 220


def lib():
    global _lib
    if _lib is not None:
        return _lib
    if not os.path.exists(LIB_PATH):
        raise ScpError(f"{LIB_PATH} is missing: run `python scp_amd/build.py` (hipcc, gfx950). "
                       "The SCP hot path has no CPU fallback.")
    L = C.CDLL(LIB_PATH)
    i32, i64 = C.c_int32, C.c_int64
    sig = {
        "scp_version": (C.c_int, []),
        "scp_geo_edge_mlps": (C.c_int, [_vp, i64, _vp, i64, _vp, i64, _vp, _vp, _vp, i64, i32, _vp]),
        "scp_mlp3_rows": (C.c_int, [_vp, i64, i64, _vp, _vp, _vp, _vp, i64, _vp, i32, i32, _vp]),
        "scp_swin_merge": (C.c_int, [_vp, i64, i64, _vp, _vp, _vp, _vp, C.c_float, _vp, i64, i32, _vp]),
        "scp_swin_ln_qkv": (C.c_int, [_vp, i64, _vp, _vp, _vp, _vp, _vp, C.c_float, _vp, i64, _vp, i64, i32, i32, _vp]),
        "scp_swin_kv_planes": (C.c_int, [_vp, _vp, i64, i64, _vp, _vp, _vp, _vp, _vp]),
        "scp_swin_attention_packed_planes": (C.c_int, [_vp, _vp, _vp, _vp, _vp, _vp, _vp, i32, i32, i32, _vp, _vp, _vp, i64, _vp, _vp]),
        "scp_split_rows_f16": (C.c_int, [_vp, i64, i32, i32, _vp, _vp, i64, _vp, _vp, _vp]),
        "scp_linear_split_f16": (C.c_int, [_vp, _vp, i64, _vp, _vp, _vp, _vp, i32, i32, _vp, _vp, i64, _vp, i64, i32, i32, i32, i32, i32, _vp]),
        "scp_last_hip_error": (C.c_int, []),
        "scp_device_count": (C.c_int, []),
        "scp_device_name": (C.c_int, [C.c_char_p, C.c_int]),
        "scp_quantize": (C.c_int, [_vp, i64, i32, C.c_double, C.c_double, _vp, _vp, C.POINTER(QuantInfo), _vp]),
        "scp_geom_create": (C.c_int, [C.POINTER(_vp)]),
        "scp_geom_destroy": (C.c_int, [_vp]),
        "scp_geom_build": (C.c_int, [_vp, _vp, i64, C.POINTER(Segment), i32, C.POINTER(SegmentInfo), _vp]),
        "scp_geom_build_xyz": (C.c_int, [_vp, _vp, _vp, i32, i32, _vp, i32, C.c_double, C.POINTER(Segment), _vp, C.POINTER(QuantInfo),
                                         C.POINTER(SegmentInfo), _vp]),
        "scp_geom_context_ehem_all": (C.c_int, [_vp, i32, i32, i32, _vp, _vp, _vp, _vp, _vp]),
        "scp_geom_emit_nodes": (C.c_int, [_vp, _vp, _vp, _vp, _vp, _vp, _vp]),
        "scp_geom_emit_leaves": (C.c_int, [_vp, i32, _vp, _vp]),
        "scp_geom_krecords_i64": (C.c_int, [_vp, i32, _vp, _vp]),
        "scp_geom_context_ehem": (C.c_int, [_vp, i32, i32, i32, _vp, _vp, _vp, _vp, _vp]),
        "scp_geom_context_octattn": (C.c_int, [_vp, i32, _vp, _vp, _vp, _vp]),
        "scp_knn_topk": (C.c_int, [_vp, i32, i32, i32, i32, _vp, _vp]),
        "scp_knn_topk_packed": (C.c_int, [_vp, _vp, i32, i32, _vp, _vp]),
        "scp_knn_topk_packed_bounded": (C.c_int, [_vp, _vp, i32, i32, _vp, _vp, _vp]),
        "scp_swin_attention_packed": (C.c_int, [_vp, _vp, _vp, _vp, _vp, i32, i32, i32, i32, _vp, _vp]),
        "scp_swin_attention_packed_split": (C.c_int, [_vp, _vp, _vp, _vp, _vp, i32, i32, i32, i32, _vp, _vp, i64, _vp]),
        "scp_set_attention_mode": (C.c_int, [i32]),
        "scp_set_attention_variant": (C.c_int, [i32]),
        "scp_get_attention_variant": (C.c_int, []),
        "scp_ctx_create": (C.c_int, [C.POINTER(_vp)]),
        "scp_ctx_destroy": (C.c_int, [_vp]),
        "scp_ctx_set": (C.c_int, [_vp, i32, i32]),
        "scp_ctx_get": (C.c_int, [_vp, i32]),
        "scp_ctx_make_current": (C.c_int, [_vp]),
        "scp_rc_debug_buffer": (C.c_int, [_vp]),
        "scp_rc_set_wide": (C.c_int, [i32]),
        "scp_prof_enable": (C.c_int, [i32]),
        "scp_prof_count": (C.c_int, []),
        "scp_prof_read": (C.c_int, [i32, _vp, _vp, _vp]),
        "scp_set_knn_mode": (C.c_int, [i32]),
        "scp_row_scale_f16": (C.c_int, [_vp, i64, i32, i32, _vp, _vp, _vp]),
        "scp_row_scale_from_max": (C.c_int, [_vp, i32, _vp, _vp, _vp]),
        "scp_linear_split_f16_max": (C.c_int, [_vp, _vp, i64, _vp, _vp, _vp, _vp, i32, i32, _vp, _vp, i64, _vp, i64, i32, i32, i32, i32, i32, _vp, _vp, i32, i32, i32, _vp]),
        "scp_octattn_attention_f16x3_vmax": (C.c_int, [_vp, _vp, _vp, _vp, _vp, i64, i32, i32, i32, i32, _vp, _vp, _vp, i64, _vp, _vp]),
        "scp_linear_f16x3_scaled": (C.c_int, [_vp, i64, _vp, _vp, _vp, i32, _vp, _vp, i64, _vp, i64, i32, i32, i32, i32, _vp, _vp, _vp]),
        "scp_layernorm_add": (C.c_int, [_vp, _vp, i64, i32, _vp, _vp, C.c_float, _vp, _vp]),
        "scp_layernorm_add_split_f16": (C.c_int, [_vp, _vp, i64, i32, _vp, _vp, C.c_float, _vp, _vp, _vp, i64, _vp, _vp, _vp]),
        "scp_set_knn_workgroup": (C.c_int, [i32]),
        "scp_knn_debug_buffer": (C.c_int, [_vp]),
        "scp_nn_sqdist_f64": (C.c_int, [_vp, i64, _vp, i64, _vp, _vp]),
        "scp_estimate_normals_f64": (C.c_int, [_vp, i64, C.c_double, i32, _vp, _vp, _vp, _vp, _vp]),
        "scp_nn_tieset_f64": (C.c_int, [i32, _vp, i64, _vp, i64, _vp, _vp, _vp, _vp]),
        "scp_edge_gather_max_ld": (C.c_int, [_vp, i64, _vp, i64, _vp, _vp, _vp, i32, i32, i32, i32, _vp, i32, _vp]),
        "scp_embed_gather": (C.c_int, [_vp, _vp, _vp, i64, _vp, _vp, _vp, _vp, _vp, _vp, i64, _vp]),
        "scp_packed_plan_sizes": (C.c_int, [_vp, i32, _vp]),
        "scp_packed_plan": (C.c_int, [_vp, i32, _vp, _vp, i32, _vp]),
        "scp_decode_expand": (C.c_int, [_vp, _vp, _vp, _vp, _vp, i64, i32, i32, i32, i32, i32, C.c_double, C.c_double, _vp, _vp, _vp, _vp, _vp, _vp, _vp]),
        "scp_edge_gather_max": (C.c_int, [_vp, _vp, _vp, _vp, _vp, i32, i32, i32, i32, _vp, i32, _vp]),
        "scp_swin_attention": (C.c_int, [_vp, _vp, _vp, _vp, i32, i32, i32, i32, i32, _vp, _vp]),
        "scp_octattn_attention": (C.c_int, [_vp, _vp, _vp, _vp, _vp, i32, i32, i32, i32, _vp, _vp, _vp]),
        "scp_octattn_f16x3_ws_bytes": (C.c_int64, [i32, i32, i32]),
        "scp_octattn_embed": (C.c_int, [_vp, _vp, i64, i32, _vp, i32, _vp, i32, i32, _vp, i32, _vp, _vp, i32, _vp, i32, _vp, _vp, _vp, i64, _vp, _vp, _vp]),
        "scp_octattn_attention_f16x3": (C.c_int, [_vp, _vp, _vp, _vp, _vp, i64, i32, i32, i32, i32, _vp, _vp, _vp, i64, _vp]),
        "scp_octattn_attention_rowinv": (C.c_int, [_vp, i64, i64, _vp, _vp, i64, i64, _vp, _vp, i64, i64, _vp, _vp, i64, i64, i32, i32, i32, i32, i32,
                                                   i32, _vp]),
        "scp_octattn_attention_rowinv_step": (C.c_int, [_vp, i64, _vp, _vp, i64, i64, i32, i32, _vp, _vp, i64, _vp, _vp, i64, _vp, _vp, i32, i32, i32,
                                                        _vp]),
        "scp_decode_expand_octattn": (C.c_int, [_vp, _vp, _vp, _vp, i64, i32, i32, i32, _vp, _vp, _vp, _vp, _vp]),
        "scp_decode_expand_batch": (C.c_int, [_vp, _vp, _vp, _vp, _vp, i64, _vp, i32, i32, _vp, i32, i64, i64, _vp, _vp, _vp, _vp, _vp, _vp, _vp, _vp]),
        "scp_split_weight_bf16": (C.c_int, [_vp, i32, i32, i32, i32, _vp, _vp, _vp]),
        "scp_linear_bf16x3": (C.c_int, [_vp, i64, _vp, _vp, i32, _vp, _vp, i64, _vp, i64, i32, i32, i32, i32, _vp]),
        "scp_split_weight_f16": (C.c_int, [_vp, i32, i32, i32, i32, _vp, _vp, _vp, _vp]),
        "scp_linear_f16x3": (C.c_int, [_vp, i64, _vp, _vp, _vp, i32, _vp, _vp, i64, _vp, i64, i32, i32, i32, i32, _vp, _vp]),
        "scp_linear_split": (C.c_int, [_vp, _vp, i64, _vp, _vp, i32, i32, _vp, _vp, i64, _vp, i64, _vp, _vp, i64, i32, i32, i32, i32, i32, _vp]),
        "scp_tile_weight_bf16": (C.c_int, [_vp, i32, i32, _vp, _vp]),
        "scp_swin_ln_linear": (C.c_int, [_vp, i64, _vp, _vp, _vp, _vp, _vp, C.c_float, _vp, i64, i32, i32, _vp]),
        "scp_swin_post_attn": (C.c_int, [_vp, _vp, i64, _vp, i64, _vp, _vp, _vp, _vp, C.c_float, _vp, i64, i32, _vp, i32, _vp]),
        "scp_swin_post_attn_weight_bytes": (C.c_int64, []),
        "scp_gelu_prescale": (C.c_double, []),
        "scp_split_rows": (C.c_int, [_vp, i64, i64, _vp, i32, _vp, _vp, i64, i64, _vp]),
        "scp_linear_split_scatter": (C.c_int, [_vp, _vp, i64, _vp, _vp, i32, i32, _vp, _vp, _vp, i64, i32, i32, i32, i32, i32, _vp]),
        "scp_linear_split_gather": (C.c_int, [_vp, _vp, i64, _vp, _vp, i32, i32, _vp, _vp, i64, _vp, _vp, i64, _vp, _vp, i64, i32, i32, i32, i32, i32, _vp]),
        "scp_linear_split_hier2": (C.c_int, [_vp, _vp, i64, i32, _vp, _vp, i64, i64, _vp, _vp, _vp, _vp, i32, _vp, _vp, _vp, i64, _vp, _vp, _vp, i64, i32, i32, i32, _vp]),
        "scp_layernorm_rows": (C.c_int, [_vp, i64, i64, _vp, _vp, i32, _vp, _vp, _vp, C.c_float, _vp, i64, i64, _vp]),
        "scp_layernorm_rows_split": (C.c_int, [_vp, i64, i64, _vp, _vp, i32, _vp, _vp, _vp, C.c_float, _vp, _vp, i64, i64, _vp]),
        "scp_gather_rows": (C.c_int, [_vp, i64, _vp, i32, _vp, i64, i64, _vp]),
        "scp_linear_f32": (C.c_int, [_vp, i64, _vp, _vp, _vp, i64, i32, i32, i32, i32, _vp]),
        "scp_softmax_cdf": (C.c_int, [_vp, i64, i64, i32, _vp, _vp, _vp, _vp, _vp]),
        "scp_pmf_cdf": (C.c_int, [_vp, i64, i32, _vp, _vp, _vp, _vp]),
        "scp_rate_workspace_bytes": (C.c_int64, [i64, i32]),
        "scp_rate_segments": (C.c_int, [_vp, i64, i64, i32, _vp, _vp, _vp, i32, _vp, _vp, _vp, _vp, i64, _vp]),
        "scp_nn_error_split_f64": (C.c_int, [_vp, i64, _vp, i64, _vp, _vp, i32, _vp, i32, _vp, _vp, _vp, _vp, _vp, _vp]),
        "scp_dist_segments_f64": (C.c_int, [_vp, _vp, _vp, _vp, i64, _vp, i32, _vp, _vp]),
        "scp_rate_leaf_share_workspace_bytes": (C.c_int64, [i64, i32]),
        "scp_rate_leaf_share": (C.c_int, [_vp, _vp, _vp, i64, _vp, _vp, _vp, i32, i64, _vp, _vp, _vp, _vp, i64, _vp]),
        "scp_ring_bins_f64": (C.c_int, [_vp, i64, _vp, _vp, i32, _vp, i32, _vp, _vp, _vp]),
        "scp_share_segments_f64": (C.c_int, [_vp, _vp, _vp, i64, _vp, i32, _vp, _vp]),
        "scp_ac_encode_cdf": (C.c_int, [_vp, _vp, i64, i32, _vp, C.c_size_t, C.POINTER(C.c_size_t)]),
        "scp_ac_encode_lohi": (C.c_int, [_vp, i64, _vp, C.c_size_t, C.POINTER(C.c_size_t)]),
        "scp_ac_dec_new": (C.c_int, [C.POINTER(_vp), _vp, C.c_size_t, i32]),
        "scp_ac_dec_next": (C.c_int, [_vp, _vp]),
        "scp_ac_dec_run": (C.c_int, [_vp, _vp, i64, _vp]),
        "scp_ac_dec_free": (C.c_int, [_vp]),
    }
    for name, (res, args) in sig.items():
        if hasattr(L, name):
            f = getattr(L, name)
            f.restype = res
            f.argtypes = args
    if L.scp_version() != ABI_VERSION:
        raise ScpError(f"{LIB_PATH} implements ABI {L.scp_version()}, this binding is written for {ABI_VERSION} (include/scp.h: "
                       "SCP_ABI_VERSION; the weight-plane layout differs between versions): rebuild with `python scp_amd/build.py`")
    _lib = L
    return L


def _check(rc, what):
    if rc < 0:
        extra = f" (hipError {lib().scp_last_hip_error()})" if rc == -4 else ""
        raise ScpError(f"{what} failed: {_ERR.get(rc, rc)}{extra}")
    return rc


_RAW_STREAM = getattr(torch._C, "_cuda_getCurrentRawStream", None)
_RAW_DEVICE = getattr(torch._C, "_cuda_getDevice", None)


def _stream():
    if _RAW_STREAM is not None and _RAW_DEVICE is not None:
        return _RAW_STREAM(_RAW_DEVICE())
    return torch.cuda.current_stream().cuda_stream


def _dev(t, dtype=None):
    if not t.is_cuda:
        raise ScpError("device tensor expected (the SCP hot path has no CPU fallback)")
    if dtype is not None and t.dtype != dtype:
# ... 196 lines not shown
                                                   _dev(wtab, torch.int32), T // 512, shift, q.stride(0), k.stride(0), o.t[0].data_ptr(),
                                                   o.t[1].data_ptr(), o.t.stride(1), _stream())
        _check(rc, "scp_swin_attention_packed_split")
        return o
    out = torch.empty((T, 256), dtype=torch.float32, device=q.device)
    rc = lib().scp_swin_attention_packed(q.data_ptr(), k.data_ptr(), v.data_ptr(), _dev(bias_table, torch.float32),
                                         _dev(wtab, torch.int32), T // 512, shift, q.stride(0), k.stride(0), _dev(out), _stream())
    _check(rc, "scp_swin_attention_packed")
    return out


class KvPlanes:

    __slots__ = ("t",)

    def __init__(self, k=None, v=None, t=None):
        if t is None:
            T = k.shape[0]
            t = torch.empty((4, T, 256), dtype=torch.bfloat16, device=k.device)
            _check(lib().scp_swin_kv_planes(k.data_ptr(), v.data_ptr(), k.stride(0), T, t[0].data_ptr(), t[1].data_ptr(), t[2].data_ptr(),
                                            t[3].data_ptr(), _stream()), "scp_swin_kv_planes")
        self.t = t


def swin_attention_packed_planes(q, kv, bias_table, wtab, shift, split=False, valid=None):
    T = q.shape[0]
    p = kv.t
    vp = None if valid is None else _dev(valid, torch.float32)
    if split:
        o = SplitAct.empty(T, 256, q.device)
        rc = lib().scp_swin_attention_packed_planes(q.data_ptr(), p[0].data_ptr(), p[1].data_ptr(), p[2].data_ptr(), p[3].data_ptr(),
                                                    _dev(bias_table, torch.float32), _dev(wtab, torch.int32), T // 512, shift, q.stride(0), None,
                                                    o.t[0].data_ptr(), o.t[1].data_ptr(), o.t.stride(1), vp, _stream())
        _check(rc, "scp_swin_attention_packed_planes")
        return o
    out = torch.empty((T, 256), dtype=torch.float32, device=q.device)
    rc = lib().scp_swin_attention_packed_planes(q.data_ptr(), p[0].data_ptr(), p[1].data_ptr(), p[2].data_ptr(), p[3].data_ptr(),
                                                _dev(bias_table, torch.float32), _dev(wtab, torch.int32), T // 512, shift, q.stride(0), _dev(out), None,
                                                None, 0, vp, _stream())
    _check(rc, "scp_swin_attention_packed_planes")
    return out


def nn_sqdist(a, b):
    a = _dev_f64(a)
    b = _dev_f64(b)
    out = torch.empty((a.shape[0],), dtype=torch.float64, device=a.device)
    _check(lib().scp_nn_sqdist_f64(a.data_ptr(), a.shape[0], b.data_ptr(), b.shape[0], out.data_ptr(), _stream()), "scp_nn_sqdist_f64")
    return out


def _dev_f64(t):
    if not t.is_cuda:
        raise ScpError("device tensor required (there is no CPU path in the product)")
    return t.to(torch.float64).contiguous()


TIE_MEAN_NORMAL, TIE_PLANE_ERROR = 0, 1


def estimate_normals(xyz, radius=1.0, max_nn=30, view=(0.0, 0.0, 0.0), want_idx=False):
    x = _dev_f64(xyz)
    n = x.shape[0]
    normals = torch.empty((n, 3), dtype=torch.float64, device=x.device)
    count = torch.empty((n,), dtype=torch.int32, device=x.device)
    idx = torch.empty((n, int(max_nn)), dtype=torch.int32, device=x.device) if want_idx else None
    v = (C.c_double * 3)(*[float(c) for c in view])
    _check(lib().scp_estimate_normals_f64(x.data_ptr(), n, float(radius), int(max_nn), C.cast(v, _vp), normals.data_ptr(), count.data_ptr(),
                                          None if idx is None else idx.data_ptr(), _stream()), "scp_estimate_normals_f64")
    return normals, count, idx


def nn_tieset(mode, q, p, dmin, nrm):
    q, p, dmin, nrm = _dev_f64(q), _dev_f64(p), _dev_f64(dmin), _dev_f64(nrm)
    nq, np_ = q.shape[0], p.shape[0]
    if nrm.shape != (np_, 3) or dmin.shape != ((np_,) if mode == TIE_MEAN_NORMAL else (nq,)):
        raise ScpError(f"nn_tieset: dmin {tuple(dmin.shape)} / normals {tuple(nrm.shape)} do not fit {nq} queries against {np_} points")
    out = torch.empty((nq, 3) if mode == TIE_MEAN_NORMAL else (nq,), dtype=torch.float64, device=q.device)
    _check(lib().scp_nn_tieset_f64(int(mode), q.data_ptr(), nq, p.data_ptr(), np_, dmin.data_ptr(), nrm.data_ptr(), out.data_ptr(), _stream()),
           "scp_nn_tieset_f64")
    return out


def embed_gather(ctx, pos, inmap, occ_enc, level_enc, octant_enc):
    rows = inmap.shape[0]
    dev = ctx.device
    x = torch.empty((rows, 80), dtype=torch.float32, device=dev)
    p = torch.empty((rows, 3), dtype=torch.float32, device=dev)
    o = torch.empty((rows,), dtype=torch.int64, device=dev)
    _check(lib().scp_embed_gather(_dev(ctx, torch.uint8), _dev(pos, torch.float32), _dev(inmap, torch.int64), ctx.shape[0], _dev(occ_enc),
                                  _dev(level_enc), _dev(octant_enc), x.data_ptr(), p.data_ptr(), o.data_ptr(), rows, _stream()),
           "scp_embed_gather")
    return x, p, o


_POPC = {}


def decode_expand(sym, pos, anc, octant, L, shift, lv_next, lv_clamp, polar, mn, den):
    dev, n = sym.device, sym.shape[0]
    tab = popcount_table(dev)
    cum = torch.cumsum(tab[sym + 1], 0)
    m = int(cum[-1])
    occ8 = torch.empty(n, dtype=torch.uint8, device=dev)
    cpos = torch.empty((m, 3), dtype=torch.int32, device=dev)
    canc = torch.empty((m, 9), dtype=torch.uint8, device=dev)
    coct = torch.empty(m, dtype=torch.uint8, device=dev)
    cctx = torch.empty((m, 12), dtype=torch.uint8, device=dev)
    cposn = torch.empty((m, 3), dtype=torch.float32, device=dev)
    if m == 0:
        return (sym + 1).clamp_(min=0).to(torch.uint8), cpos, canc, coct, cctx, cposn
    _check(lib().scp_decode_expand(_dev(sym, torch.int64), cum.data_ptr(), _dev(pos, torch.int32), _dev(anc, torch.uint8), _dev(octant, torch.uint8), n,
                                   int(L), int(shift), int(lv_next), int(lv_clamp), 1 if polar else 0, float(mn), float(den), cpos.data_ptr(), canc.data_ptr(),
                                   coct.data_ptr(), cctx.data_ptr(), cposn.data_ptr(), occ8.data_ptr(), _stream()), "scp_decode_expand")
    return occ8, cpos, canc, coct, cctx, cposn


EXPAND_SEG = np.dtype([("first", np.int64), ("count", np.int64), ("cfirst", np.int64), ("coded", np.int64), ("L", np.int32), ("shift", np.int32),
                       ("lv_next", np.int32), ("lv_clamp", np.int32), ("polar", np.int32), ("reserved", np.int32), ("mn", np.float64),
                       ("den", np.float64)])


def popcount_table(dev):
    tab = _POPC.get(dev)
    if tab is None:
        tab = _POPC[dev] = torch.tensor([bin(v).count("1") for v in range(256)], dtype=torch.int64, device=dev)
    return tab


def decode_expand_batch(sym, pos, anc, octant, cum, seg, cs, wbase, M, T):
    dev, n = sym.device, sym.shape[0]
    seg = np.ascontiguousarray(seg, EXPAND_SEG)
    wbase = np.ascontiguousarray(wbase, np.int64)
    if wbase.ndim != 2 or wbase.shape[1] != seg.shape[0]:
        raise ScpError("decode_expand_batch: wbase must be [K, S]")
    S, K, M, T = int(seg.shape[0]), int(wbase.shape[0]), int(M), int(T)
    if cum.shape[0] != n or cum.dtype != torch.int64:
        raise ScpError("decode_expand_batch: cum must be the int64 scan of the parents")
    cpos = torch.empty((M, 3), dtype=torch.int32, device=dev)
    canc = torch.empty((M, 9), dtype=torch.uint8, device=dev)
    coct = torch.empty(M, dtype=torch.uint8, device=dev)
    cctx = torch.empty((T, 12), dtype=torch.uint8, device=dev)
    cposn = torch.empty((T, 3), dtype=torch.float32, device=dev)
    if M == 0 and n > 0:
        return (sym + 1).clamp_(min=0).to(torch.uint8), cpos, canc, coct, cctx, cposn
    occ8 = torch.empty(n, dtype=torch.uint8, device=dev)
    host = torch.zeros((64 * EXPAND_SEG.itemsize + 8 * max(K * S, 1),), dtype=torch.uint8, pin_memory=True)
    host[:seg.nbytes] = torch.from_numpy(seg.view(np.uint8))
    host[64 * EXPAND_SEG.itemsize:64 * EXPAND_SEG.itemsize + wbase.nbytes] = torch.from_numpy(wbase.reshape(-1).view(np.uint8))
    scratch = host.to(dev, non_blocking=True)
    _check(lib().scp_decode_expand_batch(_dev(sym, torch.int64), cum.data_ptr(), _dev(pos, torch.int32), _dev(anc, torch.uint8), _dev(octant, torch.uint8),
                                         n, seg.ctypes.data, S, int(cs), wbase.ctypes.data, K, M, T, scratch.data_ptr(), cpos.data_ptr(),
                                         canc.data_ptr(), coct.data_ptr(), cctx.data_ptr(), cposn.data_ptr(), occ8.data_ptr(), _stream()),
           "scp_decode_expand_batch")
    return occ8, cpos, canc, coct, cctx, cposn


def packed_plan(lengths, device):
    import numpy as np
    c = np.ascontiguousarray(np.asarray(lengths, np.int64))
    W = int(c.shape[0])
    rows = np.zeros(11, np.int64)
    _check(lib().scp_packed_plan_sizes(c.ctypes.data, W, rows.ctypes.data), "scp_packed_plan_sizes")
    r = [int(x) for x in rows]
    i64, i32, f32 = torch.int64, torch.int32, torch.float32
    spec = [("inmap", i64, (r[0],)), ("a1map", i64, (r[5],)), ("a2map", i64, (r[5],)), ("even_rows", i64, (r[9],)), ("odd_rows", i64, (r[10],)),
            ("even_dst", i64, (r[9],)), ("odd_dst", i64, (r[10],))]
    for s_ in range(4):
        spec += [(f"sme{s_}", i64, (r[s_ + 1],)), (f"smo{s_}", i64, (r[s_ + 1],))]
    for s_ in range(3):
        spec += [(f"cme{s_}", i64, (r[6 + s_],)), (f"cmo{s_}", i64, (r[6 + s_],))]
    spec += [(f"sc{s_}", i64, (r[0],)) for s_ in range(1, 5)] + [(f"cc{s_}", i64, (r[5],)) for s_ in range(1, 4)]
    spec += [(f"tab{l}", i32, (r[l] // 512, 2)) for l in range(9)] + [("knn_tab", i32, (r[0] // 512, 2))]
    spec += [(f"valid{l}", f32, (r[l], 1)) for l in range(9)]
    spec += [(f"sp{s_}", i64, (r[s_],)) for s_ in range(4)] + [(f"cp{s_}", i64, (r[5 + s_],)) for s_ in range(3)]
# ... 411 lines not shown
            pb = getattr(sw, "_bias_pad", None)
            ver = (bias._version, bias.data_ptr())
            if pb is None or pb[0] is not bias or pb[2] != ver:
                pb = (bias, torch.cat((bias.detach().float(), torch.zeros(Np - N, dtype=torch.float32, device=bias.device))).contiguous(), ver)
                sw._bias_pad = pb
                note_cache_fill()
            bias = pb[1]
        N = Np
    _check(lib().scp_linear_split_scatter(t[0].data_ptr(), t[1].data_ptr(), t.stride(1), sw.tiled()[0].data_ptr(), sw.tiled()[1].data_ptr(), sw.Npad, sw.Kpad,
                                          _opt(bias), _dev(out_map, torch.int64), table.data_ptr(), table.stride(0), a.M, N, sw.K, act, cfg,
                                          _stream()), "scp_linear_split_scatter")


def split_rows(x, idx=None, out=None):
    Cc = x.shape[1]
    rows = x.shape[0] if idx is None else idx.shape[0]
    if out is None:
        out = SplitAct.empty(rows, Cc, x.device)
    if x.stride(1) != 1:
        x = x.contiguous()
    t = out.t
    _check(lib().scp_split_rows(x.data_ptr(), x.stride(0), x.shape[0], _opt(idx), Cc, t[0].data_ptr(), t[1].data_ptr(), t.stride(1), rows,
                                _stream()), "scp_split_rows")
    return out


def linear_split(a, sw, bias=None, act=ACT_NONE, residual=None, out=None, out_split=None, want="f32", cfg=0, res_map=None, res_first=False):
    M, N, K = a.M, sw.N, sw.K
    if a.K != K:
        raise ScpError("linear_split: K mismatch %d vs %d" % (a.K, K))
    t = a.t
    c = o = None
    if want in ("f32", "both"):
        c = out if out is not None else torch.empty((M, N), dtype=torch.float32, device=t.device)
    if want in ("split", "both"):
        o = out_split if out_split is not None else SplitAct.empty(M, N, t.device)
    r2 = residual
    if res_map is not None or res_first:
        rc = lib().scp_linear_split_gather(t[0].data_ptr(), t[1].data_ptr(), t.stride(1), sw.tiled()[0].data_ptr(), sw.tiled()[1].data_ptr(), sw.Npad, sw.Kpad,
                                           _opt(bias), None if r2 is None else r2.data_ptr(), 0 if r2 is None else r2.stride(0),
                                           None if res_map is None else _dev(res_map, torch.int64),
                                           None if c is None else c.data_ptr(), 0 if c is None else c.stride(0),
                                           None if o is None else o.t[0].data_ptr(), None if o is None else o.t[1].data_ptr(),
                                           0 if o is None else o.t.stride(1), M, N, K, act, cfg, _stream())
        _check(rc, "scp_linear_split_gather")
        return c if want == "f32" else (o if want == "split" else (c, o))
    rc = lib().scp_linear_split(t[0].data_ptr(), t[1].data_ptr(), t.stride(1), sw.tiled()[0].data_ptr(), sw.tiled()[1].data_ptr(), sw.Npad, sw.Kpad, _opt(bias),
                                None if r2 is None else r2.data_ptr(), 0 if r2 is None else r2.stride(0),
                                None if c is None else c.data_ptr(), 0 if c is None else c.stride(0),
                                None if o is None else o.t[0].data_ptr(), None if o is None else o.t[1].data_ptr(),
                                0 if o is None else o.t.stride(1), M, N, K, act, cfg, _stream())
    _check(rc, "scp_linear_split")
    return c if want == "f32" else (o if want == "split" else (c, o))


def linear_split_hier2(a0, sw0, a1, sw1, parent, bias=None, act=ACT_NONE, residual=None, res_map=None, out_split=None):
    if not WTILE:
        raise ScpError("linear_split_hier2 reads tiled weight planes (SCP_WTILE=0 is not supported by it)")
    M, N = a0.M, sw0.N
    if a0.K != sw0.K or a1.K != sw1.K or sw1.K != 256 or sw1.N != N or sw1.Npad != sw0.Npad or parent.shape[0] != M:
        raise ScpError("linear_split_hier2: operand shapes do not match")
    o = out_split if out_split is not None else SplitAct.empty(M, N, a0.t.device)
    t0, t1 = a0.t, a1.t
    rc = lib().scp_linear_split_hier2(t0[0].data_ptr(), t0[1].data_ptr(), t0.stride(1), sw0.Kpad, t1[0].data_ptr(), t1[1].data_ptr(), t1.stride(1), a1.M,
                                      sw0.tiled()[0].data_ptr(), sw0.tiled()[1].data_ptr(), sw1.tiled()[0].data_ptr(), sw1.tiled()[1].data_ptr(), sw0.Npad,
                                      _dev(parent, torch.int64), _opt(bias), None if residual is None else residual.data_ptr(),
                                      0 if residual is None else residual.stride(0), None if (residual is None or res_map is None) else _dev(res_map, torch.int64),
                                      o.t[0].data_ptr(), o.t[1].data_ptr(), o.t.stride(1), M, N, act, _stream())
    _check(rc, "scp_linear_split_hier2")
    return o


class LnFoldedWeight:

    def __init__(self, w, gamma, beta):
        w64 = w.detach().double()
        self.sw = SplitWeight((w64 * gamma.detach().double()[None, :]).float())
        self.planes = _tiled_planes_always(self.sw)
        self.wbeta = (w64 @ beta.detach().double()).float().contiguous()
        self.N, self.K = self.sw.N, self.sw.K
        note_cache_fill()


def swin_ln_linear(x, fw, bias, eps=1e-5, valid=None, out=None):
    M = x.shape[0]
    if x.shape[1] != 256 or fw.K != 256 or x.stride(1) != 1:
        raise ScpError("swin_ln_linear: 256-channel rows expected")
    if out is None:
        out = torch.empty((M, fw.N), dtype=torch.float32, device=x.device)
    t = fw.planes
    rc = lib().scp_swin_ln_linear(x.data_ptr(), x.stride(0), None if valid is None else _dev(valid, torch.float32), t[0].data_ptr(), t[1].data_ptr(),
                                  _opt(bias), _dev(fw.wbeta), float(eps), out.data_ptr(), out.stride(0), M, fw.N, _stream())
    _check(rc, "scp_swin_ln_linear")
    return out


def swin_ln_qkv(x, fw, bias, eps=1e-5, valid=None):
    M = x.shape[0]
    if x.shape[1] != 256 or fw.K != 256 or x.stride(1) != 1 or fw.N not in (512, 768) or (M & 127):
        raise ScpError("swin_ln_qkv: 256-channel rows in multiples of 128, N = 768 or 512 expected")
    q = torch.empty((M, 256), dtype=torch.float32, device=x.device) if fw.N == 768 else None
    pl = torch.empty((4, M, 256), dtype=torch.bfloat16, device=x.device)
    t = fw.planes
    rc = lib().scp_swin_ln_qkv(x.data_ptr(), x.stride(0), None if valid is None else _dev(valid, torch.float32), t[0].data_ptr(), t[1].data_ptr(),
                               _opt(bias), _dev(fw.wbeta), float(eps), None if q is None else q.data_ptr(), 256, pl.data_ptr(), M, M, fw.N, _stream())
    _check(rc, "scp_swin_ln_qkv")
    return q, KvPlanes(t=pl)


class EdgeMlpWeights:

    def __init__(self, mlp1, mlp2):
        w11, w12, w13 = (mlp1[i].weight.detach().float() for i in (0, 2, 4))
        w21, w22, w23 = (mlp2[i].weight.detach().float() for i in (0, 2, 4))
        if tuple(w11.shape) != (256, 448) or tuple(w12.shape) != (256, 256) or tuple(w13.shape) != (256, 256) or tuple(w21.shape) != (256, 512) or \
                tuple(w22.shape) != (256, 256) or tuple(w23.shape) != (128, 256):
            raise ScpError("EdgeMlpWeights: unexpected layer shapes")
        dev = w11.device
        P = rc_perm16(256, dev)
        z = torch.zeros((256, 64), dtype=torch.float32, device=dev)
        mats = [w11[:, :256], torch.cat((w11[:, 256:], z), 1), w12[:, P], w13[:, P], w21[:, 256:][:, P], w21[:, :256], w22[:, P],
                torch.cat((w23[:, P], torch.zeros((128, 256), dtype=torch.float32, device=dev)), 0)]
        nbytes = lib().scp_swin_post_attn_weight_bytes()
        buf = torch.zeros((nbytes // 2,), dtype=torch.bfloat16, device=dev)
        half = nbytes // 4
        for m, w in enumerate(mats):
            hi, lo = _tiled_planes_always(SplitWeight(w.contiguous()))
            buf[m * 65536:(m + 1) * 65536] = hi.reshape(-1)[:65536]
            buf[half + m * 65536:half + (m + 1) * 65536] = lo.reshape(-1)[:65536]
        self.packed = buf
        self.bias = torch.cat([mlp1[i].bias.detach().float() for i in (0, 2, 4)] + [mlp2[i].bias.detach().float() for i in (0, 2, 4)]).contiguous()
        note_cache_fill()


def geo_edge_mlps(pos1, pos2, pos3, ew, out):
    M = pos1.shape[0]
    if pos1.shape[1] != 64 or pos2.shape[1] != 128 or pos3.shape[1] != 256 or pos1.stride(1) != 1 or pos2.stride(1) != 1 or pos3.stride(1) != 1 or out.stride(1) != 1:
        raise ScpError("geo_edge_mlps: [M, 64], [M, 128], [M, 256] rows expected")
    rc = lib().scp_geo_edge_mlps(pos1.data_ptr(), pos1.stride(0), pos2.data_ptr(), pos2.stride(0), pos3.data_ptr(), pos3.stride(0), ew.packed.data_ptr(),
                                 ew.bias.data_ptr(), out.data_ptr(), out.stride(0), M, _stream())
    _check(rc, "scp_geo_edge_mlps")
    return out


class Mlp3Weights:

    def __init__(self, seq):
        ws = [seq[i].weight.detach().float() for i in (0, 2, 4)]
        bs = [seq[i].bias.detach().float() for i in (0, 2, 4)]
        if ws[0].shape[1] != 256 or any(w.shape[0] > 256 or w.shape[1] > 256 for w in ws) or ws[1].shape[1] != ws[0].shape[0] or ws[2].shape[1] != ws[1].shape[0]:
            raise ScpError("Mlp3Weights: a 256 -> (<= 256) -> (<= 256) -> (<= 256) head expected")
        dev = ws[0].device
        P = rc_perm16(256, dev)
        nbytes = lib().scp_swin_post_attn_weight_bytes()
        buf = torch.zeros((nbytes // 2,), dtype=torch.bfloat16, device=dev)
        half = nbytes // 4
        bias = torch.zeros((3, 256), dtype=torch.float32, device=dev)
        for m, (w, b) in enumerate(zip(ws, bs)):
            full = torch.zeros((256, 256), dtype=torch.float32, device=dev)
            full[:w.shape[0], :w.shape[1]] = w
            if m:
                full = full[:, P]
            hi, lo = _tiled_planes_always(SplitWeight(full.contiguous()))
            buf[m * 65536:(m + 1) * 65536] = hi.reshape(-1)[:65536]
            buf[half + m * 65536:half + (m + 1) * 65536] = lo.reshape(-1)[:65536]
            bias[m, :b.shape[0]] = b
# ... 62 lines not shown
        tiles = [_tiled_planes_always(w) for w in (swp, sw1, sw2)]
        self.packed = torch.cat([t[0].reshape(-1) for t in tiles] + [t[1].reshape(-1) for t in tiles]).contiguous()
        if self.packed.numel() * 2 != lib().scp_swin_post_attn_weight_bytes():
            raise ScpError("swin_post_attn: 256 -> 1024 -> 256 blocks only")
        self.bp = bp.detach().float().contiguous()
        self.b1 = ((b1.detach().double() + w1d @ beta.detach().double()) * s).float().contiguous()
        self.b2 = b2.detach().float().contiguous()
        note_cache_fill()


def swin_post_attn(o, x, pw, eps=1e-5, out=None, tiles=None):
    M = x.shape[0]
    if o.K != 256 or o.M != M or x.shape[1] != 256 or x.stride(1) != 1:
        raise ScpError("swin_post_attn: [M, 256] operands expected")
    if out is None:
        out = torch.empty((M, 256), dtype=torch.float32, device=x.device)
    t = o.t
    rc = lib().scp_swin_post_attn(t[0].data_ptr(), t[1].data_ptr(), t.stride(1), x.data_ptr(), x.stride(0), pw.packed.data_ptr(), _dev(pw.bp),
                                  _dev(pw.b1), _dev(pw.b2), float(eps), out.data_ptr(), out.stride(0), M,
                                  None if tiles is None else _dev(tiles, torch.int32), 0 if tiles is None else int(tiles.shape[0]), _stream())
    _check(rc, "scp_swin_post_attn")
    return out


def layernorm_rows(x, gamma, beta, eps=1e-5, valid=None, ia=None, ib=None, out=None, split=False):
    Cc = gamma.shape[0]
    rows = x.shape[0] if ia is None else ia.shape[0]
    if split:
        o = SplitAct.empty(rows, Cc, x.device)
        rc = lib().scp_layernorm_rows_split(x.data_ptr(), x.stride(0), x.shape[0], None if ia is None else _dev(ia, torch.int64),
                                            None if ib is None else _dev(ib, torch.int64), Cc, _dev(gamma), _dev(beta),
                                            None if valid is None else _dev(valid, torch.float32), float(eps), o.t[0].data_ptr(),
                                            o.t[1].data_ptr(), o.t.stride(1), rows, _stream())
        _check(rc, "scp_layernorm_rows_split")
        return o
    if out is None:
        out = torch.empty((rows, Cc), dtype=torch.float32, device=x.device)
    rc = lib().scp_layernorm_rows(x.data_ptr(), x.stride(0), x.shape[0], None if ia is None else _dev(ia, torch.int64),
                                  None if ib is None else _dev(ib, torch.int64), Cc, _dev(gamma), _dev(beta),
                                  None if valid is None else _dev(valid, torch.float32), float(eps), out.data_ptr(), out.stride(0),
                                  rows, _stream())
    _check(rc, "scp_layernorm_rows")
    return out


def layernorm_add(a, b, gamma, beta, eps=1e-5, planes=False):
    Cc = a.shape[-1]
    if not a.is_contiguous() or (b is not None and (not b.is_contiguous() or b.shape != a.shape)):
        raise ScpError("layernorm_add: contiguous operands of one shape expected")
    out = torch.empty_like(a)
    if planes:
        M, ld = a.numel() // Cc, -(-Cc // 32) * 32
        pl = torch.empty((2, M, ld), dtype=torch.float16, device=a.device)
        ws = torch.empty((2, M), dtype=torch.float32, device=a.device)
        _check(lib().scp_layernorm_add_split_f16(_dev(a, torch.float32), None if b is None else _dev(b, torch.float32), M, Cc, _dev(gamma), _dev(beta),
                                                 float(eps), out.data_ptr(), pl[0].data_ptr(), pl[1].data_ptr(), ld, ws[0].data_ptr(), ws[1].data_ptr(),
                                                 _stream()), "scp_layernorm_add_split_f16")
        return out, SplitActF16(parts=(pl[0], pl[1], ws[0], ws[1], Cc))
    _check(lib().scp_layernorm_add(_dev(a, torch.float32), None if b is None else _dev(b, torch.float32), a.numel() // Cc, Cc, _dev(gamma), _dev(beta),
                                   float(eps), out.data_ptr(), _stream()), "scp_layernorm_add")
    return out


def gather_rows(src, idx, out):
    Cc = out.shape[1]
    rc = lib().scp_gather_rows(src.data_ptr(), src.stride(0), _dev(idx, torch.int64), Cc, out.data_ptr(), out.stride(0), idx.shape[0],
                               _stream())
    _check(rc, "scp_gather_rows")
    return out


def linear_f32(x, w, bias=None, act=ACT_NONE):
    K = w.shape[1]
    N = w.shape[0]
    lead = x.shape[:-1]
    x2 = x.reshape(-1, K) if x.is_contiguous() else x.contiguous().reshape(-1, K)
    M = x2.shape[0]
    out = torch.empty((M, N), dtype=torch.float32, device=x.device)
    wc = w if w.is_contiguous() else w.contiguous()
    rc = lib().scp_linear_f32(x2.data_ptr(), x2.stride(0), _dev(wc.detach(), torch.float32), _opt(bias), out.data_ptr(), N, M, N, K, act,
                              _stream())
    _check(rc, "scp_linear_f32")
    return out.reshape(*lead, N)


OCTATTN_MODE = os.environ.get("SCP_OCTATTN", "f16x3")


def octattn_attention(q_u, k, k_u, v, v_u, heads, out=None, out_u=None, vmax=None):
    B, c, D = q_u.shape
    if out is None:
        out, out_u = torch.empty_like(q_u), torch.empty_like(q_u)
    elif not (out.is_contiguous() and out_u.is_contiguous() and out.shape == q_u.shape and out_u.shape == q_u.shape):
        raise ScpError("octattn_attention: out / out_u must be contiguous [B, c, D] float32")
    hd = D // heads
    ld = k.stride(-2)
    strided_ok = all(t.is_cuda and t.dtype == torch.float32 and t.stride(-1) == 1 and t.stride(-2) == ld and (t.dim() == 2 or t.stride(0) == c * ld)
                     for t in (k, k_u, v, v_u))
    if OCTATTN_MODE == "f16x3" and hd == 150 and (D & 3) == 0 and strided_ok:
        nb = lib().scp_octattn_f16x3_ws_bytes(B, c, heads)
        ws = torch.empty((nb + 1024,), dtype=torch.uint8, device=q_u.device)
        off = (-ws.data_ptr()) % 1024
        if vmax is not None:
            rc = lib().scp_octattn_attention_f16x3_vmax(_dev(q_u), k.data_ptr(), k_u.data_ptr(), v.data_ptr(), v_u.data_ptr(), ld, B, c, heads, hd, _dev(out),
                                                        _dev(out_u), ws.data_ptr() + off, nb, _dev(vmax, torch.int32), _stream())
            _check(rc, "scp_octattn_attention_f16x3_vmax")
            return out, out_u
        rc = lib().scp_octattn_attention_f16x3(_dev(q_u), k.data_ptr(), k_u.data_ptr(), v.data_ptr(), v_u.data_ptr(), ld, B, c, heads, hd, _dev(out),
                                               _dev(out_u), ws.data_ptr() + off, nb, _stream())
        _check(rc, "scp_octattn_attention_f16x3")
        return out, out_u
    k, k_u, v, v_u = (t.contiguous() for t in (k, k_u, v, v_u))
    rc = lib().scp_octattn_attention(_dev(q_u), _dev(k), _dev(k_u), _dev(v), _dev(v_u), B, c, heads, hd,
                                     _dev(out), _dev(out_u), _stream())
    _check(rc, "scp_octattn_attention")
    return out, out_u


def _win_strides(t):
    if not (t.is_cuda and t.dtype == torch.float32 and t.stride(-1) == 1):
        raise ScpError("octattn_attention_rowinv: float32 device tensors with unit channel stride expected")
    return (t.stride(0) if t.dim() == 3 else 0), t.stride(-2)


def octattn_attention_rowinv(q_u, k, v, heads, k_u=None, v_u=None, out=None, out_u=None, q0=0, q1=None, qoff=0):
    D = q_u.shape[-1]
    B = q_u.shape[0] if q_u.dim() == 3 else 1
    q1 = (q_u.shape[-2] + qoff) if q1 is None else q1
    if out is None and out_u is None:
        raise ScpError("octattn_attention_rowinv: nothing to compute (out and out_u are None)")
    if q1 > k.shape[-2] or q1 - qoff > q_u.shape[-2]:
        raise ScpError("octattn_attention_rowinv: query range beyond the key rows")
    for t in (out, out_u, k_u, v_u):
        if t is not None and t.shape[-2] < q1 - qoff:
            raise ScpError("octattn_attention_rowinv: operand shorter than the query range")
    qw, qr = _win_strides(q_u)
    kw, kr = _win_strides(k)
    if _win_strides(v) != (kw, kr):
        raise ScpError("octattn_attention_rowinv: k and v must share their strides")
    uw = ur = 0
    if out_u is not None:
        uw, ur = _win_strides(k_u)
        if _win_strides(v_u) != (uw, ur):
            raise ScpError("octattn_attention_rowinv: k_u and v_u must share their strides")
    ow, orr = _win_strides(out if out is not None else out_u)
    if out is not None and out_u is not None and _win_strides(out_u) != (ow, orr):
        raise ScpError("octattn_attention_rowinv: out and out_u must share their strides")
    ptr = lambda t: None if t is None else t.data_ptr()
    rc = lib().scp_octattn_attention_rowinv(q_u.data_ptr(), qw, qr, k.data_ptr(), v.data_ptr(), kw, kr, ptr(k_u), ptr(v_u), uw, ur, ptr(out),
                                            ptr(out_u), ow, orr, B, int(q0), int(q1), int(qoff), int(heads), D // heads, _stream())
    _check(rc, "scp_octattn_attention_rowinv")
    return out, out_u


def octattn_attention_rowinv_step(q_u, k, v, t, slot, heads, k_u=None, v_u=None, out=None, out_u=None):
    if out is None and out_u is None:
        raise ScpError("octattn_attention_rowinv_step: nothing to compute (out and out_u are None)")
    if q_u.dim() != 2 or k.dim() != 3 or v.shape != k.shape or k.shape[-1] != q_u.shape[-1]:
        raise ScpError("octattn_attention_rowinv_step: q_u [S, D] and k, v [slots, rows, D] expected")
    S, D = q_u.shape
    for x in (t, slot):
        if not (x.is_cuda and x.dtype == torch.int32 and x.dim() == 1 and x.is_contiguous()):
            raise ScpError("octattn_attention_rowinv_step: t and slot are contiguous int32 device tensors")
    if t.shape[0] != k.shape[0] or slot.shape[0] != S:
        raise ScpError("octattn_attention_rowinv_step: t has one entry per cache slot, slot one per launch row")
    if out_u is not None and (k_u is None or v_u is None):
# ... 342 lines not shown
```

Measured before the change: 15.81 frames/s.

## Fuse geometry mlp2 three-layer MLP into one kernel and gather embeddings in place

Adds a single HIP kernel that runs the 80-80-64-64 leaky MLP with intermediates kept in LDS, replacing three separate fp32 GEMM launches. The embedding gather gets a leading-dimension variant so it writes straight into the concatenated edge-conv feature buffer, and the MLP output goes directly into the next concat buffer, removing two copy kernels. The diff also carries refactoring of the fp32 GEMM into shared helpers and partial lnlin2 mode and pad-fast hooks, which look unrelated to the speed change. The fused kernel is specialised to the fixed widths and uses extra LDS per block, which may lower occupancy.

```diff
diff --git a/include/scp.h b/include/scp.h
--- a/include/scp.h
+++ b/include/scp.h
@@ -174,6 +174,8 @@
 
 SCP_API int scp_linear_f32(const float *A, int64_t lda, const float *W, const float *bias, float *C, int64_t ldc, int32_t M, int32_t N, int32_t K,
                    int32_t act, void *stream);
+SCP_API int scp_geo_mlp2_f32(const float *A, int64_t lda, const float *W1, const float *b1, const float *W2, const float *b2, const float *W3,
+                   const float *b3, float *C, int64_t ldc, int32_t M, int32_t K0, int32_t H1, int32_t H2, int32_t N, void *stream);
 
 SCP_API int scp_octattn_attention(const float *q_u, const float *k, const float *k_u, const float *v, const float *v_u,
                           int32_t B, int32_t c, int32_t H, int32_t hd, float *out, float *out_u, void *stream);
@@ -275,6 +277,9 @@
 SCP_API int scp_embed_gather(const uint8_t *ctx, const float *pos, const int64_t *inmap, int64_t n_tokens, const float *occ_enc,
                      const float *level_enc, const float *octant_enc, float *x, float *pos_out, int64_t *occ_self, int64_t rows,
                      void *stream);
+SCP_API int scp_embed_gather_ld(const uint8_t *ctx, const float *pos, const int64_t *inmap, int64_t n_tokens, const float *occ_enc,
+                     const float *level_enc, const float *octant_enc, float *x, int64_t ldx, float *pos_out, int64_t *occ_self, int64_t rows,
+                     void *stream);
 
 SCP_API int scp_packed_plan_sizes(const int64_t *lengths, int32_t W, int64_t *rows_out);
 SCP_API int scp_packed_plan(const int64_t *lengths, int32_t W, int64_t *tables_dev, void *const *outs, int32_t n_outs, void *stream);
diff --git a/include/scp_debug.h b/include/scp_debug.h
--- a/include/scp_debug.h
+++ b/include/scp_debug.h
@@ -16,6 +16,8 @@
 SCP_API int scp_get_attention_variant(void);
 SCP_API int scp_rc_set_grid(int32_t workgroups);
 SCP_API int scp_rc_set_wide(int32_t mode);
+SCP_API int scp_lnlin2_set_mode(int32_t mode);
+SCP_API int scp_lnlin2_set_pad_fast(int32_t on);
 
 enum {
     SCP_PROF_POST_ATTN = 1,
diff --git a/scp_amd/csrc/fused.hip b/scp_amd/csrc/fused.hip
--- a/scp_amd/csrc/fused.hip
+++ b/scp_amd/csrc/fused.hip
@@ -230,8 +230,8 @@
 __global__ __launch_bounds__(256) void embed_gather_kernel(const unsigned char *__restrict__ ctx, const float *__restrict__ pos,
                                                           const int64_t *__restrict__ inmap, int64_t n_tokens, const float *__restrict__ occ_enc,
                                                           const float *__restrict__ level_enc, const float *__restrict__ octant_enc,
-                                                          float *__restrict__ x, float *__restrict__ pos_out, int64_t *__restrict__ occ_self,
-                                                          int64_t rows) {
+                                                          float *__restrict__ x, int64_t ldx, float *__restrict__ pos_out,
+                                                          int64_t *__restrict__ occ_self, int64_t rows) {
     const int64_t g = (int64_t)blockIdx.x * 256 + threadIdx.x;
     if (g >= rows * 20) return;
     const int64_t r = g / 20;
@@ -251,7 +251,7 @@
         const int oc = pad ? 0 : c[3 * (p - 16) + 1];
         v = *(const f32x4 *)(octant_enc + oc * 4);
     }
-    *(f32x4 *)(x + r * 80 + 4 * p) = v;
+    *(f32x4 *)(x + r * ldx + 4 * p) = v;
     if (p == 0) {
         occ_self[r] = pad ? 255 : c[11];
         pos_out[3 * r] = pad ? 0.f : pos[3 * t];
@@ -260,15 +260,21 @@
     }
 }
 
+extern "C" SCP_API int scp_embed_gather_ld(const uint8_t *ctx, const float *pos, const int64_t *inmap, int64_t n_tokens, const float *occ_enc,
+                                           const float *level_enc, const float *octant_enc, float *x, int64_t ldx, float *pos_out, int64_t *occ_self,
+                                           int64_t rows, void *stream) {
+    if (!ctx || !pos || !inmap || !occ_enc || !level_enc || !octant_enc || !x || !pos_out || !occ_self || rows < 0 || n_tokens <= 0 || ldx < 80 ||
+        (ldx & 3) || (((uintptr_t)occ_enc | (uintptr_t)level_enc | (uintptr_t)octant_enc | (uintptr_t)x) & 15))
+        return SCP_EINVAL;
+    if (rows == 0) return SCP_OK;
+    hipLaunchKernelGGL(embed_gather_kernel, dim3((unsigned)cdiv64(rows * 20, 256)), dim3(256), 0, (hipStream_t)stream, ctx, pos, inmap, n_tokens,
+                       occ_enc, level_enc, octant_enc, x, ldx, pos_out, occ_self, rows);
+    LAUNCH_CHECK();
+    return SCP_OK;
+}
+
 extern "C" SCP_API int scp_embed_gather(const uint8_t *ctx, const float *pos, const int64_t *inmap, int64_t n_tokens, const float *occ_enc,
                                         const float *level_enc, const float *octant_enc, float *x, float *pos_out, int64_t *occ_self,
                                         int64_t rows, void *stream) {
-    if (!ctx || !pos || !inmap || !occ_enc || !level_enc || !octant_enc || !x || !pos_out || !occ_self || rows < 0 || n_tokens <= 0 ||
-        (((uintptr_t)occ_enc | (uintptr_t)level_enc | (uintptr_t)octant_enc | (uintptr_t)x) & 15))
-        return SCP_EINVAL;
-    if (rows == 0) return SCP_OK;
-    hipLaunchKernelGGL(embed_gather_kernel, dim3((unsigned)cdiv64(rows * 20, 256)), dim3(256), 0, (hipStream_t)stream, ctx, pos, inmap, n_tokens,
-                       occ_enc, level_enc, octant_enc, x, pos_out, occ_self, rows);
-    LAUNCH_CHECK();
-    return SCP_OK;
-}
+    return scp_embed_gather_ld(ctx, pos, inmap, n_tokens, occ_enc, level_enc, octant_enc, x, 80, pos_out, occ_self, rows, stream);
+}
diff --git a/scp_amd/csrc/gemm.hip b/scp_amd/csrc/gemm.hip
--- a/scp_amd/csrc/gemm.hip
+++ b/scp_amd/csrc/gemm.hip
@@ -401,6 +401,30 @@
 #define FBK 32
 #define FLD 36
 
+__device__ __forceinline__ void f32_stage_piece(float *d, int pc, const f32x4 v) {
+    const int o = pc >> 1;
+    *(float2 *)(d + o) = make_float2(v[0], v[2]);
+    *(float2 *)(d + 16 + o) = make_float2(v[1], v[3]);
+}
+template <int NB>
+__device__ __forceinline__ void f32_ktile_mfma(const float *ar, const float *br, f32x16 (&acc)[NB]) {
+#pragma unroll
+    for (int g = 0; g < 4; ++g) {
+        const f32x4 a = *(const f32x4 *)(ar + 4 * g);
+#pragma unroll
+        for (int j = 0; j < NB; ++j) {
+            const f32x4 b = *(const f32x4 *)(br + j * 32 * FLD + 4 * g);
+            acc[j] = __builtin_amdgcn_mfma_f32_32x32x2f32(a[0], b[0], acc[j], 0, 0, 0);
+            acc[j] = __builtin_amdgcn_mfma_f32_32x32x2f32(a[1], b[1], acc[j], 0, 0, 0);
+            acc[j] = __builtin_amdgcn_mfma_f32_32x32x2f32(a[2], b[2], acc[j], 0, 0, 0);
+            acc[j] = __builtin_amdgcn_mfma_f32_32x32x2f32(a[3], b[3], acc[j], 0, 0, 0);
+        }
+    }
+}
+template <int ACT>
+__device__ __forceinline__ float f32_epilogue(float acc, float bv) { return apply_act<ACT>(acc + bv); }
+__device__ __forceinline__ int f32_acc_row(int r, int h) { return (r & 3) + 8 * (r >> 2) + 4 * h; }
+
 template <int ACT>
 __global__ __launch_bounds__(256, 2) void gemm_f32_kernel(const float *__restrict__ A, int64_t lda, const float *__restrict__ W,
                                                          const float *__restrict__ bias, float *__restrict__ C, int64_t ldc, int M, int N, int K) {
@@ -437,19 +461,10 @@
         }
     };
     auto store_tile = [&]() {
-        const int o = pc >> 1;
-#pragma unroll
-        for (int i = 0; i < 4; ++i) {
-            float *d = sA + (pr + 32 * i) * FLD;
-            *(float2 *)(d + o) = make_float2(ra[i][0], ra[i][2]);
-            *(float2 *)(d + 16 + o) = make_float2(ra[i][1], ra[i][3]);
-        }
-#pragma unroll
-        for (int i = 0; i < 2; ++i) {
-            float *d = sB + (pr + 32 * i) * FLD;
-            *(float2 *)(d + o) = make_float2(rb[i][0], rb[i][2]);
-            *(float2 *)(d + 16 + o) = make_float2(rb[i][1], rb[i][3]);
-        }
+#pragma unroll
+        for (int i = 0; i < 4; ++i) f32_stage_piece(sA + (pr + 32 * i) * FLD, pc, ra[i]);
+#pragma unroll
+        for (int i = 0; i < 2; ++i) f32_stage_piece(sB + (pr + 32 * i) * FLD, pc, rb[i]);
     };
     if (vec) load_tile(0);
     for (int kt = 0; kt < nk; ++kt) {
@@ -471,19 +486,7 @@
         }
         __syncthreads();
         if (vec && kt + 1 < nk) load_tile(kt + 1);
-        const float *ar = sA + (w * 32 + col) * FLD + h * 16;
-#pragma unroll
-        for (int g = 0; g < 4; ++g) {
-            const f32x4 a = *(const f32x4 *)(ar + 4 * g);
-#pragma unroll
-            for (int j = 0; j < 2; ++j) {
-                const f32x4 b = *(const f32x4 *)(sB + (j * 32 + col) * FLD + h * 16 + 4 * g);
-                acc[j] = __builtin_amdgcn_mfma_f32_32x32x2f32(a[0], b[0], acc[j], 0, 0, 0);
-                acc[j] = __builtin_amdgcn_mfma_f32_32x32x2f32(a[1], b[1], acc[j], 0, 0, 0);
-                acc[j] = __builtin_amdgcn_mfma_f32_32x32x2f32(a[2], b[2], acc[j], 0, 0, 0);
-                acc[j] = __builtin_amdgcn_mfma_f32_32x32x2f32(a[3], b[3], acc[j], 0, 0, 0);
-            }
-        }
+        f32_ktile_mfma<2>(sA + (w * 32 + col) * FLD + h * 16, sB + col * FLD + h * 16, acc);
     }
 #pragma unroll
     for (int j = 0; j < 2; ++j) {
@@ -492,8 +495,8 @@
         const float bv = bias ? bias[n] : 0.f;
 #pragma unroll
         for (int r = 0; r < 16; ++r) {
-            const int m = m0 + w * 32 + (r & 3) + 8 * (r >> 2) + 4 * h;
-            if (m < M) C[(int64_t)m * ldc + n] = apply_act<ACT>(acc[j][r] + bv);
+            const int m = m0 + w * 32 + f32_acc_row(r, h);
+            if (m < M) C[(int64_t)m * ldc + n] = f32_epilogue<ACT>(acc[j][r], bv);
         }
     }
 }
@@ -509,3 +512,103 @@
     LAUNCH_CHECK();
     return SCP_OK;
 }
+
+#define GM_K0 80
+#define GM_H1 80
+#define GM_H2 64
+#define GM_N 64
+#define GM_XT (FBM * FLD)
+#define GM_LDS ((3 * GM_XT + 96 * FLD) * 4)
+
+struct GeoMlp3Args {
+    const float *A; int64_t lda;
+    const float *W1, *b1, *W2, *b2, *W3, *b3;
+    float *C; int64_t ldc;
+    int M;
+};
+
+template <int K, int N, int ACT, bool LAST>
+__device__ __forceinline__ void gm_layer(const GeoMlp3Args &a, const float *__restrict__ W, const float *__restrict__ bias, float *sX, float *sW, int m0) {
+    constexpr int NK = (K + FBK - 1) / FBK, NB = (N + 31) / 32;
+    const int tid = threadIdx.x, w = tid >> 6, lane = tid & 63, col = lane & 31, h = lane >> 5;
+    const int pr = tid >> 3, pc = (tid & 7) * 4;
+    f32x16 acc[NB];
+#pragma unroll
+    for (int j = 0; j < NB; ++j)
+#pragma unroll
+        for (int r = 0; r < 16; ++r) acc[j][r] = 0.f;
+    f32x4 rb[NB];
+    auto load_w = [&](int kt) {
+        const int kk = kt * FBK + pc;
+        const bool kin = kk < K;
+#pragma unroll
+        for (int i = 0; i < NB; ++i) {
+            const int n = pr + 32 * i;
+            const f32x4 v = *(const f32x4 *)(W + (n < N ? n : N - 1) * K + (kin ? kk : 0));
+            rb[i] = (kin && n < N) ? v : (f32x4){0.f, 0.f, 0.f, 0.f};
+        }
+    };
+    load_w(0);
+#pragma unroll
+    for (int kt = 0; kt < NK; ++kt) {
+        __syncthreads();
+#pragma unroll
+        for (int i = 0; i < NB; ++i) f32_stage_piece(sW + (pr + 32 * i) * FLD, pc, rb[i]);
+        __syncthreads();
+        if (kt + 1 < NK) load_w(kt + 1);
+        f32_ktile_mfma<NB>(sX + kt * GM_XT + (w * 32 + col) * FLD + h * 16, sW + col * FLD + h * 16, acc);
+    }
+#pragma unroll
+    for (int j = 0; j < NB; ++j) {
+        const int n = j * 32 + col;
+        const float bv = (bias && n < N) ? bias[n] : 0.f;
+#pragma unroll
+        for (int r = 0; r < 16; ++r) {
+            const int rl = w * 32 + f32_acc_row(r, h);
+            if (LAST) {
+                if (n < N && m0 + rl < a.M) a.C[(int64_t)(m0 + rl) * a.ldc + n] = f32_epilogue<ACT>(acc[j][r], bv);
+            } else {
+                sX[j * GM_XT + rl * FLD + (col & 1) * 16 + (col >> 1)] = n < N ? f32_epilogue<ACT>(acc[j][r], bv) : 0.f;
+            }
+        }
+    }
+}
+
+__global__ __launch_bounds__(256, 2) void geo_mlp3_f32_kernel(const GeoMlp3Args a) {
+    extern __shared__ __attribute__((aligned(16))) float gm_smem[];
+    float *sX = gm_smem, *sW = gm_smem + 3 * GM_XT;
+    const int tid = threadIdx.x, pr = tid >> 3, pc = (tid & 7) * 4;
+    const int m0 = blockIdx.x * FBM;
+#pragma unroll
+    for (int kt = 0; kt < 3; ++kt) {
+        const int kk = kt * FBK + pc;
+        const bool kin = kk < GM_K0;
+#pragma unroll
+        for (int i = 0; i < 4; ++i) {
+            const int m = m0 + pr + 32 * i;
+            const f32x4 v = *(const f32x4 *)(a.A + (int64_t)(m < a.M ? m : a.M - 1) * a.lda + (kin ? kk : 0));
+            f32_stage_piece(sX + kt * GM_XT + (pr + 32 * i) * FLD, pc, (kin && m < a.M) ? v : (f32x4){0.f, 0.f, 0.f, 0.f});
+        }
+    }
+    gm_layer<GM_K0, GM_H1, ACT_LEAKY, false>(a, a.W1, a.b1, sX, sW, m0);
+    gm_layer<GM_H1, GM_H2, ACT_LEAKY, false>(a, a.W2, a.b2, sX, sW, m0);
+    gm_layer<GM_H2, GM_N, ACT_NONE, true>(a, a.W3, a.b3, sX, sW, m0);
+}
+
+extern "C" SCP_API int scp_geo_mlp2_f32(const float *A, int64_t lda, const float *W1, const float *b1, const float *W2, const float *b2, const float *W3,
+                                        const float *b3, float *C, int64_t ldc, int32_t M, int32_t K0, int32_t H1, int32_t H2, int32_t N, void *stream) {
+    if (!A || !W1 || !W2 || !W3 || !C || M <= 0 || K0 != GM_K0 || H1 != GM_H1 || H2 != GM_H2 || N != GM_N || lda < K0 || (lda & 3) || ldc < N ||
+        (((uintptr_t)A | (uintptr_t)W1 | (uintptr_t)W2 | (uintptr_t)W3) & 15))
+        return SCP_EINVAL;
+    static bool configured = false;
+    if (!configured) {
+        HIP_TRY(hipFuncSetAttribute((const void *)geo_mlp3_f32_kernel, hipFuncAttributeMaxDynamicSharedMemorySize, GM_LDS));
+        configured = true;
+    }
+    GeoMlp3Args a;
+    a.A = A; a.lda = lda; a.W1 = W1; a.b1 = b1; a.W2 = W2; a.b2 = b2; a.W3 = W3; a.b3 = b3; a.C = C; a.ldc = ldc; a.M = M;
+    SCP_PROF(SCP_PROF_GEMM_F32, stream, 2.0 * M * (double)(GM_K0 * GM_H1 + GM_H1 * GM_H2 + GM_H2 * GM_N));
+    hipLaunchKernelGGL(geo_mlp3_f32_kernel, dim3((unsigned)((M + FBM - 1) / FBM)), dim3(256), GM_LDS, (hipStream_t)stream, a);
+    LAUNCH_CHECK();
+    return SCP_OK;
+}
diff --git a/scp_amd/csrc/lnlin2.hip b/scp_amd/csrc/lnlin2.hip
--- a/scp_amd/csrc/lnlin2.hip
+++ b/scp_amd/csrc/lnlin2.hip
@@ -113,6 +113,71 @@
         for (int it = 0; it < 4; ++it)
             __builtin_amdgcn_raw_buffer_store_b128(y[plane][it], prs, L.lane * 16, it * 1024 + (vblk + head) * 4096 + (2 + plane) * pbytes, 0);
     asm volatile("s_waitcnt lgkmcnt(0)" ::: "memory");
+}
+
+template <bool KV>
+__device__ __forceinline__ void l2_bias_start(unsigned atb, unsigned atv, unsigned maskh, int j, int nq, rf32x16 &c0, rf32x16 &c1) {
+    if (KV && j >= nq + 4) {
+        float bb[2], bwv[2];
+        const unsigned ad = atv + 256 * j;
+        asm volatile("ds_read_b32 %0, %4\n\tds_read_b32 %1, %4 offset:128\n\tds_read_b32 %2, %4 offset:4096\n\tds_read_b32 %3, %4 offset:4224\n\t"
+                     "s_waitcnt lgkmcnt(0)" : "=&v"(bb[0]), "=&v"(bb[1]), "=&v"(bwv[0]), "=&v"(bwv[1]) : "v"(ad) : "memory");
+#pragma unroll
+        for (int blk = 0; blk < 2; ++blk) {
+            rf32x16 &c = blk ? c1 : c0;
+#pragma unroll
+            for (int r = 0; r < 16; ++r) c[r] = ((maskh >> (8 * (r >> 2) + (r & 3))) & 1u) ? bwv[blk] : bb[blk];
+        }
+    } else {
+        const unsigned ad = atb + 256 * j;
+        rf32x4 t[2][4];
+        L2_READ4(t[0][0], t[0][1], t[0][2], t[0][3], ad, 0, 32, 64, 96);
+        L2_READ4(t[1][0], t[1][1], t[1][2], t[1][3], ad, 128, 160, 192, 224);
+#pragma unroll
+        for (int q = 0; q < 4; ++q)
+#pragma unroll
+            for (int u = 0; u < 4; ++u) { c0[4 * q + u] = t[0][q][u]; c1[4 * q + u] = t[1][q][u]; }
+    }
+}
+
+struct L2TileOut {
+    __amdgpu_buffer_rsrc_t rs;
+    int kvoff, vblk;
+};
+__device__ __forceinline__ L2TileOut l2_tile_out(const RcLane &L, const RcLnLinArgs &a, int m0) {
+    L2TileOut t;
+    const int64_t rows_left = (int64_t)a.M - m0;
+    const int64_t span = (rows_left < RC_ROWS ? rows_left : RC_ROWS) * a.ldo * 4;
+    t.rs = __builtin_amdgcn_make_buffer_rsrc(a.out + (int64_t)m0 * a.ldo, 0, (a.probe & 1) ? 0 : (int)span, 0x00020000);
+    t.kvoff = (m0 + 32 * L.w + (L.lane >> 3)) * 512 + (L.lane & 7) * 16;
+    t.vblk = ((m0 >> 5) + L.w) * 4;
+    return t;
+}
+
+template <bool KV, bool SW>
+__device__ __forceinline__ void l2_store_step(const RcLane &L, char *bounce, const rf32x16 &c0, const rf32x16 &c1, const L2TileOut &t,
+                                              __amdgpu_buffer_rsrc_t prs, int ldo_bytes, int voff, int pbytes, int j, int nq) {
+    if (!SW && j < nq) {
+#pragma unroll
+        for (int blk = 0; blk < 2; ++blk) {
+            rf32x4 o[4];
+#pragma unroll
+            for (int q = 0; q < 4; ++q)
+#pragma unroll
+                for (int u = 0; u < 4; ++u) o[q][u] = (blk ? c1 : c0)[4 * q + u];
+            rc_store_block(L, bounce, o, t.rs, ldo_bytes, voff, 64 * j + 32 * blk);
+        }
+    } else if (!SW) {
+        l2_store_k(L, bounce, c0, c1, prs, t.kvoff, pbytes, j - nq);
+    } else {
+        l2_store_v(L, bounce, c0, c1, prs, t.vblk, pbytes, j - nq - 4);
+    }
+}
+
+__device__ __forceinline__ bool l2_valid_pair(const RcLnLinArgs &a, int tile, int lane) {
+    const int64_t r = (int64_t)tile * RC_ROWS + lane;
+    const float v0 = r < a.M ? a.valid[r] : 0.f, v1 = r + 64 < a.M ? a.valid[r + 64] : 0.f;
+    return v0 != 0.f || v1 != 0.f;
 }
 
 template <bool KV>
@@ -144,8 +209,28 @@
     __syncthreads();
     int slot = 0;
     if (dma) { l2_issue(L, wr_hi, wr_lo, 0, 0, smem); l2_issue(L, wr_hi, wr_lo, 0, 1, smem + L2_Q); }
+    const bool pad_fast = a.pad_fast && a.valid;
+    const unsigned atv = asb + 4 * L.col;
+    bool live = pad_fast ? l2_valid_pair(a, blockIdx.x, L.lane) : true;
     for (int tile = blockIdx.x; tile < ntiles; tile += (int)gridDim.x) {
         const int m0 = tile * RC_ROWS;
+        if (pad_fast) {
+            const bool pad = __builtin_amdgcn_ballot_w64(live) == 0;
+            live = l2_valid_pair(a, tile + (int)gridDim.x, L.lane);
+            if (pad) {
+                const L2TileOut to = l2_tile_out(L, a, m0);
+                const rbf16x8 z = __builtin_bit_cast(rbf16x8, (ru32x4){0u, 0u, 0u, 0u});
+                rf32x16 c0, c1;
+                for (int j = 0; j < nsteps; ++j) {
+                    l2_bias_start<KV>(asb + 16 * L.h, atv, 0u, j, nq, c0, c1);
+                    c0 = __builtin_amdgcn_mfma_f32_32x32x16_bf16(z, z, c0, 0, 0, 0);
+                    c1 = __builtin_amdgcn_mfma_f32_32x32x16_bf16(z, z, c1, 0, 0, 0);
+                    if (KV && j >= nq + 4) l2_store_step<KV, true>(L, bounce, c0, c1, to, prs, ldo_bytes, voff, pbytes, j, nq);
+                    else l2_store_step<KV, false>(L, bounce, c0, c1, to, prs, ldo_bytes, voff, pbytes, j, nq);
+                }
+                continue;
+            }
+        }
         const int row = m0 + 32 * L.w + L.col;
         const int rowc = row < a.M ? row : a.M - 1;
         float keep = (row < a.M) ? 1.0f : 0.0f;
@@ -172,39 +257,12 @@
             }
         }
         const bool kept = keep != 0.f;
-        const int64_t rows_left = (int64_t)a.M - m0;
-        const int64_t span = (rows_left < RC_ROWS ? rows_left : RC_ROWS) * a.ldo * 4;
-        const __amdgpu_buffer_rsrc_t rs = __builtin_amdgcn_make_buffer_rsrc(a.out + (int64_t)m0 * a.ldo, 0, (a.probe & 1) ? 0 : (int)span, 0x00020000);
+        const L2TileOut to = l2_tile_out(L, a, m0);
         const unsigned kmask = (unsigned)__builtin_amdgcn_ballot_w64(kept);
         const unsigned maskh = kmask >> (4 * L.h);
-        const int kvoff = (m0 + 32 * L.w + (L.lane >> 3)) * 512 + (L.lane & 7) * 16;
-        const int vblk = ((m0 >> 5) + L.w) * 4;
-
-        const unsigned atb = asb + (kept ? 4096 : 0) + 16 * L.h, atv = asb + 4 * L.col;
+        const unsigned atb = asb + (kept ? 4096 : 0) + 16 * L.h;
         rf32x16 c0, c1;
-        auto bias_start = [&](int j) {
-            if (KV && j >= nq + 4) {
-                float bb[2], bwv[2];
-                const unsigned ad = atv + 256 * j;
-                asm volatile("ds_read_b32 %0, %4\n\tds_read_b32 %1, %4 offset:128\n\tds_read_b32 %2, %4 offset:4096\n\tds_read_b32 %3, %4 offset:4224\n\t"
-                             "s_waitcnt lgkmcnt(0)" : "=&v"(bb[0]), "=&v"(bb[1]), "=&v"(bwv[0]), "=&v"(bwv[1]) : "v"(ad) : "memory");
-#pragma unroll
-                for (int blk = 0; blk < 2; ++blk) {
-                    rf32x16 &c = blk ? c1 : c0;
-#pragma unroll
-                    for (int r = 0; r < 16; ++r) c[r] = ((maskh >> (8 * (r >> 2) + (r & 3))) & 1u) ? bwv[blk] : bb[blk];
-                }
-            } else {
-                const unsigned ad = atb + 256 * j;
-                rf32x4 t[2][4];
-                L2_READ4(t[0][0], t[0][1], t[0][2], t[0][3], ad, 0, 32, 64, 96);
-                L2_READ4(t[1][0], t[1][1], t[1][2], t[1][3], ad, 128, 160, 192, 224);
-#pragma unroll
-                for (int q = 0; q < 4; ++q)
-#pragma unroll
-                    for (int u = 0; u < 4; ++u) { c0[4 * q + u] = t[0][q][u]; c1[4 * q + u] = t[1][q][u]; }
-            }
-        };
+        auto bias_start = [&](int j) { l2_bias_start<KV>(atb, atv, maskh, j, nq, c0, c1); };
         bias_start(0);
         SCP_WAIT_DMA(0);
         auto steps = [&](auto sw, int ja, int jb) {
@@ -227,21 +285,7 @@
             L2_QUARTER(3, 4)
 #undef L2_QUARTER
             __builtin_amdgcn_sched_barrier(0);
-            if (!SW && j < nq) {
-#pragma unroll
-                for (int blk = 0; blk < 2; ++blk) {
-                    rf32x4 o[4];
-#pragma unroll
-                    for (int q = 0; q < 4; ++q)
-#pragma unroll
-                        for (int u = 0; u < 4; ++u) o[q][u] = (blk ? c1 : c0)[4 * q + u];
-                    rc_store_block(L, bounce, o, rs, ldo_bytes, voff, 64 * j + 32 * blk);
-                }
-            } else if (!SW) {
-                l2_store_k(L, bounce, c0, c1, prs, kvoff, pbytes, j - nq);
-            } else {
-                l2_store_v(L, bounce, c0, c1, prs, vblk, pbytes, j - nq - 4);
-            }
+            l2_store_step<KV, SW>(L, bounce, c0, c1, to, prs, ldo_bytes, voff, pbytes, j, nq);
             if (j + 1 < nsteps) bias_start(jn);
         }
         };
@@ -251,11 +295,17 @@
     SCP_WAIT_DMA(0);
 }
 
+static int g_l2_mode = -1, g_l2_pad = -1;
 int scp_lnlin2_mode() {
-    static int mode = -1;
-    if (mode < 0) { const char *e = getenv("SCP_LNLIN"); mode = e ? atoi(e) : 0; if (mode < 0 || mode > 2) mode = 0; }
-    return mode;
-}
+    if (g_l2_mode < 0) { const char *e = getenv("SCP_LNLIN"); g_l2_mode = e ? atoi(e) : 0; if (g_l2_mode < 0 || g_l2_mode > 2) g_l2_mode = 0; }
+    return g_l2_mode;
+}
+extern "C" SCP_API int scp_lnlin2_set_mode(int32_t mode) { g_l2_mode = (mode < 0 || mode > 2) ? 0 : mode; return SCP_OK; }
+static int l2_pad_fast() {
+    if (g_l2_pad < 0) { const char *e = getenv("SCP_LNPAD"); g_l2_pad = (e && e[0] == '0') ? 0 : 1; }
+    return g_l2_pad;
+}
+extern "C" SCP_API int scp_lnlin2_set_pad_fast(int32_t on) { g_l2_pad = on ? 1 : 0; return SCP_OK; }
 
 int scp_lnlin2_launch(RcLnLinArgs a, bool kv, int ncu, hipStream_t stream) {
     static int one = -1, probe = -1;
@@ -267,7 +317,7 @@
         HIP_TRY(hipFuncSetAttribute((const void *)ln2_proj_kernel<true>, hipFuncAttributeMaxDynamicSharedMemorySize, one ? L2_LDS_ONE : L2_LDS));
         configured = true;
     }
-    a.ngroups = 1; a.probe = probe; a.dbg = nullptr;
+    a.ngroups = 1; a.probe = probe; a.dbg = nullptr; a.pad_fast = l2_pad_fast();
     const int ntiles = (a.M + RC_ROWS - 1) / RC_ROWS;
     const int wgs = (one ? 1 : 2) * ncu;
     const dim3 grid((unsigned)(ntiles < wgs ? ntiles : wgs));
diff --git a/scp_amd/csrc/rc_common.h b/scp_amd/csrc/rc_common.h
--- a/scp_amd/csrc/rc_common.h
+++ b/scp_amd/csrc/rc_common.h
@@ -94,6 +94,7 @@
     unsigned long long *dbg;
     __bf16 *planes; int64_t plane_bytes; int nq;
     int ngroups;
+    int pad_fast;
 };
 
 int scp_lnlin2_mode();
diff --git a/scp_amd/csrc/rowchain.hip b/scp_amd/csrc/rowchain.hip
--- a/scp_amd/csrc/rowchain.hip
+++ b/scp_amd/csrc/rowchain.hip
@@ -1499,7 +1499,7 @@
     RcLnLinArgs a;
     a.x = x; a.ldx = ldx; a.valid = valid; a.Whi = (const __bf16 *)Whi; a.Wlo = (const __bf16 *)Wlo; a.bias = bias; a.wbeta = wbeta;
     a.out = out; a.ldo = ldo; a.M = M; a.N = N; a.eps = eps;
-    a.planes = nullptr; a.plane_bytes = 0; a.nq = 0;
+    a.planes = nullptr; a.plane_bytes = 0; a.nq = 0; a.pad_fast = 0;
     { static int pr = -1; if (pr < 0) { const char *e = getenv("SCP_RC_PROBE"); pr = e ? atoi(e) : 0; } a.probe = pr; }
     if (a.probe) { const char *e = getenv("SCP_RC_PROBE"); a.probe = e ? atoi(e) : 0; }
     a.dbg = g_rc_dbg;
@@ -1527,7 +1527,7 @@
     RcLnLinArgs a;
     a.x = x; a.ldx = ldx; a.valid = valid; a.Whi = (const __bf16 *)Whi; a.Wlo = (const __bf16 *)Wlo; a.bias = bias; a.wbeta = wbeta;
     a.out = q; a.ldo = q ? ldq : 256; a.M = M; a.N = N; a.eps = eps; a.probe = 0; a.dbg = nullptr;
-    a.planes = (__bf16 *)planes; a.plane_bytes = Tp * 512; a.nq = N / 64 - 8;
+    a.planes = (__bf16 *)planes; a.plane_bytes = Tp * 512; a.nq = N / 64 - 8; a.pad_fast = 0;
     const int ntiles = M / RC_ROWS, ncu = rc_num_cu();
     SCP_PROF(SCP_PROF_LN_LINEAR, stream, 2.0 * M * 256.0 * N);
     if (rc_lnlin2_here(ntiles, ncu)) return scp_lnlin2_launch(a, true, ncu, (hipStream_t)stream);
diff --git a/scp_amd/models/packed.py b/scp_amd/models/packed.py
--- a/scp_amd/models/packed.py
+++ b/scp_amd/models/packed.py
@@ -277,6 +277,9 @@
     _head3(model, "prob_pred_mlp1", a, out=table, out_map=out_map)
 
 
+GEO_FUSED = __import__("os").environ.get("SCP_GEOMLP", "fused") != "split"
+
+
 @torch.no_grad()
 def ehem_phase1_packed(model, ctx, pos, plan, table=None):
     d = plan.d
@@ -284,9 +287,14 @@
     dev = ctx.device
     fused_in = (ctx.dtype == torch.uint8 and g.occ_enc.weight.shape[1] == 16 and g.level_enc.weight.shape[1] == 4
                 and g.octant_enc.weight.shape[1] == 4)
+    c1, c2 = g.conv1[0].weight.shape[0], g.conv2[0].weight.shape[0]
+    nx0, nx1 = g.mlp2[0].weight.shape[1], g.mlp2[4].weight.shape[0]
+    in_place = GEO_FUSED and fused_in
     if fused_in:
-        x, pos0, occ_self = native.embed_gather(ctx, pos, d["inmap"], g.occ_enc.weight, g.level_enc.weight, g.octant_enc.weight)
-        P0 = x.shape[0]
+        P0 = d["inmap"].shape[0]
+        f2 = torch.empty((P0, c1 + nx0), dtype=torch.float32, device=dev)
+        x, pos0, occ_self = native.embed_gather(ctx, pos, d["inmap"], g.occ_enc.weight, g.level_enc.weight, g.octant_enc.weight,
+                                                out=f2[:, c1:] if in_place else None)
     else:
         pad_ctx = torch.tensor([[0, 0, 255] * 4], dtype=ctx.dtype, device=dev)
         ctx0 = torch.cat((ctx, pad_ctx))[d["inmap"]].long()
@@ -296,14 +304,17 @@
                        F.embedding(ctx0[:, 0::3], g.level_enc.weight).reshape(P0, -1),
                        F.embedding(ctx0[:, 1::3], g.octant_enc.weight).reshape(P0, -1)), 1)
         occ_self = ctx0[:, 11]
+        f2 = torch.empty((P0, c1 + x.shape[1]), dtype=torch.float32, device=dev)
     ktab = d["knn_tab"]
-    c1, c2 = g.conv1[0].weight.shape[0], g.conv2[0].weight.shape[0]
-    f2 = torch.empty((P0, c1 + x.shape[1]), dtype=torch.float32, device=dev)
-    f2[:, c1:] = x
+    if not in_place:
+        f2[:, c1:] = x
     pos1 = _edge_conv_packed(g.conv1, pos0, ktab, out=f2[:, :c1])
-    x = leaky_mlp3(g.mlp2, x, exact=True)
-    f3 = torch.empty((P0, c2 + x.shape[1]), dtype=torch.float32, device=dev)
-    f3[:, c2:] = x
+    f3 = torch.empty((P0, c2 + nx1), dtype=torch.float32, device=dev)
+    if in_place:
+        x = native.geo_mlp2_f32(g.mlp2, x, out=f3[:, c2:])
+    else:
+        x = leaky_mlp3(g.mlp2, x, exact=True)
+        f3[:, c2:] = x
     pos2 = _edge_conv_packed(g.conv2, f2, ktab, out=f3[:, :c2])
     pos3 = _edge_conv_packed(g.conv3, f3, ktab, feeds_knn=False)
     nx = g.mlp3[4].weight.shape[0]
diff --git a/scp_amd/native.py b/scp_amd/native.py
--- a/scp_amd/native.py
+++ b/scp_amd/native.py
@@ -88,6 +88,8 @@
         "scp_ctx_make_current": (C.c_int, [_vp]),
         "scp_rc_debug_buffer": (C.c_int, [_vp]),
         "scp_rc_set_wide": (C.c_int, [i32]),
+        "scp_lnlin2_set_mode": (C.c_int, [i32]),
+        "scp_lnlin2_set_pad_fast": (C.c_int, [i32]),
         "scp_prof_enable": (C.c_int, [i32]),
         "scp_prof_count": (C.c_int, []),
         "scp_prof_read": (C.c_int, [i32, _vp, _vp, _vp]),
@@ -106,6 +108,8 @@
         "scp_nn_tieset_f64": (C.c_int, [i32, _vp, i64, _vp, i64, _vp, _vp, _vp, _vp]),
         "scp_edge_gather_max_ld": (C.c_int, [_vp, i64, _vp, i64, _vp, _vp, _vp, i32, i32, i32, i32, _vp, i32, _vp]),
         "scp_embed_gather": (C.c_int, [_vp, _vp, _vp, i64, _vp, _vp, _vp, _vp, _vp, _vp, i64, _vp]),
+        "scp_embed_gather_ld": (C.c_int, [_vp, _vp, _vp, i64, _vp, _vp, _vp, _vp, i64, _vp, _vp, i64, _vp]),
+        "scp_geo_mlp2_f32": (C.c_int, [_vp, i64, _vp, _vp, _vp, _vp, _vp, _vp, _vp, i64, i32, i32, i32, i32, i32, _vp]),
         "scp_packed_plan_sizes": (C.c_int, [_vp, i32, _vp]),
         "scp_packed_plan": (C.c_int, [_vp, i32, _vp, _vp, i32, _vp]),
         "scp_decode_expand": (C.c_int, [_vp, _vp, _vp, _vp, _vp, i64, i32, i32, i32, i32, i32, C.c_double, C.c_double, _vp, _vp, _vp, _vp, _vp, _vp, _vp]),
@@ -468,15 +472,18 @@
     return out
 
 
-def embed_gather(ctx, pos, inmap, occ_enc, level_enc, octant_enc):
+def embed_gather(ctx, pos, inmap, occ_enc, level_enc, octant_enc, out=None):
     rows = inmap.shape[0]
     dev = ctx.device
-    x = torch.empty((rows, 80), dtype=torch.float32, device=dev)
+    x = torch.empty((rows, 80), dtype=torch.float32, device=dev) if out is None else out
+    if tuple(x.shape) != (rows, 80) or x.dtype != torch.float32 or x.stride(1) != 1:
+        raise ScpError("embed_gather: out must be fp32 [rows, 80] with unit column stride")
     p = torch.empty((rows, 3), dtype=torch.float32, device=dev)
     o = torch.empty((rows,), dtype=torch.int64, device=dev)
-    _check(lib().scp_embed_gather(_dev(ctx, torch.uint8), _dev(pos, torch.float32), _dev(inmap, torch.int64), ctx.shape[0], _dev(occ_enc),
-                                  _dev(level_enc), _dev(octant_enc), x.data_ptr(), p.data_ptr(), o.data_ptr(), rows, _stream()),
-           "scp_embed_gather")
+    _check(lib().scp_embed_gather_ld(_dev(ctx, torch.uint8), _dev(pos, torch.float32), _dev(inmap, torch.int64), ctx.shape[0], _dev(occ_enc),
+                                     _dev(level_enc), _dev(octant_enc), x.data_ptr(), x.stride(0) if rows > 1 else max(x.stride(0), 80), p.data_ptr(),
+                                     o.data_ptr(), rows, _stream()),
+           "scp_embed_gather_ld")
     return x, p, o
 
 
@@ -1054,6 +1061,14 @@
         note_cache_fill()
 
 
+def set_lnlin_mode(mode):
+    _check(lib().scp_lnlin2_set_mode(int(mode)), "scp_lnlin2_set_mode")
+
+
+def set_lnlin_pad_fast(on):
+    _check(lib().scp_lnlin2_set_pad_fast(1 if on else 0), "scp_lnlin2_set_pad_fast")
+
+
 def swin_ln_linear(x, fw, bias, eps=1e-5, valid=None, out=None):
     M = x.shape[0]
     if x.shape[1] != 256 or fw.K != 256 or x.stride(1) != 1:
@@ -1282,6 +1297,24 @@
                               _stream())
     _check(rc, "scp_linear_f32")
     return out.reshape(*lead, N)
+
+
+def geo_mlp2_f32(seq, x, out=None):
+    w = [seq[i].weight.detach() for i in (0, 2, 4)]
+    M = x.shape[0]
+    if x.dim() != 2 or x.dtype != torch.float32 or x.stride(1) != 1 or x.shape[1] != w[0].shape[1] or w[1].shape[1] != w[0].shape[0] or w[2].shape[1] != w[1].shape[0]:
+        raise ScpError("geo_mlp2_f32: fp32 rows with unit column stride, widths chained through the three layers expected")
+    N = w[2].shape[0]
+    if out is None:
+        out = torch.empty((M, N), dtype=torch.float32, device=x.device)
+    if tuple(out.shape) != (M, N) or out.dtype != torch.float32 or out.stride(1) != 1:
+        raise ScpError("geo_mlp2_f32: out must be fp32 [M, N] with unit column stride")
+    ld = lambda t: t.stride(0) if M > 1 else max(t.stride(0), t.shape[1])
+    rc = lib().scp_geo_mlp2_f32(x.data_ptr(), ld(x), _dev(w[0], torch.float32), _opt(seq[0].bias), _dev(w[1], torch.float32), _opt(seq[2].bias),
+                                _dev(w[2], torch.float32), _opt(seq[4].bias), out.data_ptr(), ld(out), M, w[0].shape[1], w[0].shape[0], w[1].shape[0], N,
+                                _stream())
+    _check(rc, "scp_geo_mlp2_f32")
+    return out
 
 
 OCTATTN_MODE = os.environ.get("SCP_OCTATTN", "f16x3")
```

New measurement: 15.81 frames/s. About the same (-0.0%).
